# iclavera/learning_to_adapt

Hardware: AMD Instinct MI355X
Metric: controller-steps/sec (n_cand=2000, H=30, ens=5) (higher is better)
Workload: dtype f32

## Files before the change

include/l2a.h:

```cpp
#ifndef L2A_H_
#define L2A_H_

#ifdef __cplusplus
extern "C" {
#endif

typedef struct l2a_ctx l2a_ctx;
typedef struct l2a_model l2a_model;
typedef struct l2a_lstm l2a_lstm;
typedef struct l2a_reward_model l2a_reward_model;
typedef struct l2a_value_model l2a_value_model;
typedef struct l2a_policy_model l2a_policy_model;
typedef struct l2a_controller l2a_controller;

#define L2A_OK 0
#define L2A_EINVAL (-1)
#define L2A_EHIP (-2)
#define L2A_ENODEV (-3)
#define L2A_ESTATE (-4)
#define L2A_ESPLIT (-5)

#define L2A_ACT_IDENTITY 0
#define L2A_ACT_RELU 1
#define L2A_ACT_TANH 2
#define L2A_ACT_SIGMOID 3
#define L2A_ACT_SWISH 4

#define L2A_MODE_SINGLE 0
#define L2A_MODE_PER_BLOCK 1
#define L2A_MODE_MEAN 2

#define L2A_KERNEL_AUTO 0
#define L2A_KERNEL_MFMA 1
#define L2A_KERNEL_VALU 2

typedef struct l2a_reward {
    float w_vel;
    float inv_dt;
    float alive;
    float ctrl_coef;
    float dist_coef;
    int vel_index;
    int dist_index;
    int reserved;
} l2a_reward;

#define L2A_PROGRAM_MAX_TERMS 16
#define L2A_PROGRAM_MAX_CONSTS 64
#define L2A_SRC_OBS 0
#define L2A_SRC_ACT 1
#define L2A_SRC_NEXT 2
#define L2A_SRC_DELTA 3
#define L2A_TERM_LINEAR 0
#define L2A_TERM_SQSUM 1
#define L2A_TERM_NORM 2
#define L2A_TERM_INRANGE 3
typedef struct l2a_reward_term {
    int kind;
    int source;
    int index;
    int len;
    int target;
    float coef;
    float lo;
    float hi;
} l2a_reward_term;
typedef struct l2a_reward_program {
    int n_terms;
    int n_consts;
    float bias;
    int reserved;
    l2a_reward_term terms[L2A_PROGRAM_MAX_TERMS];
    float consts[L2A_PROGRAM_MAX_CONSTS];
} l2a_reward_program;

int l2a_init(int device, l2a_ctx** out);
void l2a_destroy(l2a_ctx* ctx);
const char* l2a_last_error(const l2a_ctx* ctx);
int l2a_device_info(const l2a_ctx* ctx, char* buf, int cap);
int l2a_set_kernel(l2a_ctx* ctx, int kind);
int l2a_set_split(l2a_ctx* ctx, int policy);
int l2a_set_batch(l2a_ctx* ctx, int sets);
int l2a_set_xcd_align(l2a_ctx* ctx, int on);
int l2a_set_fan(l2a_ctx* ctx, int on);
int l2a_set_double_rounds(l2a_ctx* ctx, int on);
int l2a_set_micro(l2a_ctx* ctx, int policy);
int l2a_launch_status(l2a_ctx* ctx, int* status_out);
int l2a_set_spin_limit(l2a_ctx* ctx, unsigned int polls);
int l2a_inject_status(l2a_ctx* ctx, int bits);
int l2a_set_debug_buffer(l2a_ctx* ctx, void* device_ptr);

int l2a_model_create(l2a_ctx* ctx, int obs_dim, int act_dim, int n_hidden, const int* hidden,
                     int hidden_act, int output_act, int n_sets, int mode, l2a_model** out);
void l2a_model_destroy(l2a_model* model);

int l2a_model_set_weights(l2a_model* model, int e, const void* const* device_ptrs,
                          void* stream);

int l2a_model_set_norm(l2a_model* model, int e, const double* mean_obs, const double* std_obs,
                       const double* mean_act, const double* std_act,
                       const double* mean_delta, const double* std_delta, void* stream);

int l2a_plan_rs(l2a_model* model, const float* obs0, const float* actions, int m, int n, int h,
                double discount, const l2a_reward* reward, int cand_offset, float* returns_out,
                unsigned long long* best_key, void* stream);

int l2a_plan_rs_sync(l2a_model* model, const float* obs_host, const float* actions, int m, int n, int h,
                     double discount, const l2a_reward* reward, int cand_offset, float* returns_out,
                     unsigned long long* keys_host_out, void* stream);

int l2a_plan_rs_chunk(l2a_model* model, const float* state, int state_per_row, const float* actions, int m, int n,
                      int h_chunk, int t0, double discount, const l2a_reward* reward, int cand_offset,
                      const float* returns_in, float* returns_out, float* state_out, unsigned long long* best_key,
                      void* stream);

int l2a_reward_program_check(const l2a_reward_program* program, int obs_dim, int act_dim);
int l2a_score_trajectory(l2a_ctx* ctx, const float* obs0, const float* traj, const float* actions, int m, int n, int h,
                         int obs_dim, int act_dim, double discount, const l2a_reward_program* program, int cand_offset,
                         float* returns_out, unsigned long long* best_key, void* stream);
int l2a_plan_rs_program(l2a_model* model, const float* obs0, const float* actions, int m, int n, int h, double discount,
                        const l2a_reward_program* program, int cand_offset, float* returns_out,
                        unsigned long long* best_key, float* traj_out, void* stream);

int l2a_reward_model_check(int obs_dim, int act_dim, int n_hidden, const int* hidden, int hidden_act);
int l2a_reward_model_geometry(int obs_dim, int act_dim, int n_hidden, const int* hidden, long long rows, int h, int num_cu,
                              int lds_per_block, int* out);
int l2a_reward_model_create(l2a_ctx* ctx, int obs_dim, int act_dim, int n_hidden, const int* hidden, int hidden_act,
                            l2a_reward_model** out);
void l2a_reward_model_destroy(l2a_reward_model* rm);
int l2a_reward_model_set_weights(l2a_reward_model* rm, const void* const* device_ptrs, void* stream);
int l2a_reward_model_set_norm(l2a_reward_model* rm, const double* mean_obs, const double* std_obs, const double* mean_act,
                              const double* std_act, const double* mean_delta, const double* std_delta, const double* mean_r,
                              const double* std_r, void* stream);
int l2a_reward_model_predict(l2a_reward_model* rm, const float* obs, const float* act, const float* next_obs, int rows,
                             float* rewards_out, void* stream);
int l2a_score_trajectory_model(l2a_reward_model* rm, const float* obs0, const float* traj, const float* actions, int m, int n,
                               int h, double discount, int cand_offset, float* returns_out, unsigned long long* best_key,
                               void* stream);
int l2a_plan_rs_reward_model(l2a_model* model, l2a_reward_model* rm, const float* obs0, const float* actions, int m, int n,
                             int h, double discount, int cand_offset, float* returns_out, unsigned long long* best_key,
                             float* traj_out, void* stream);

int l2a_value_model_check(int obs_dim, int n_hidden, const int* hidden, int hidden_act);
int l2a_value_model_geometry(int obs_dim, int n_hidden, const int* hidden, long long rows, int num_cu, int lds_per_block,
                             int* out);
int l2a_value_model_create(l2a_ctx* ctx, int obs_dim, int n_hidden, const int* hidden, int hidden_act, l2a_value_model** out);
void l2a_value_model_destroy(l2a_value_model* vm);
int l2a_value_model_set_weights(l2a_value_model* vm, const void* const* device_ptrs, void* stream);
int l2a_value_model_set_norm(l2a_value_model* vm, const double* mean_obs, const double* std_obs, const double* mean_v,
                             const double* std_v, void* stream);
int l2a_value_model_predict(l2a_value_model* vm, const float* states, int rows, float* values_out, void* stream);
int l2a_value_terminal(l2a_value_model* vm, const float* final_state, const float* returns_in, int m, int n, int h,
                       double discount, double value_coef, int cand_offset, float* returns_out, unsigned long long* best_key,
                       void* stream);
int l2a_plan_rs_value(l2a_model* model, l2a_value_model* vm, const float* obs0, const float* actions, int m, int n, int h,
                      double discount, const l2a_reward* reward, double value_coef, int cand_offset, float* returns_out,
                      unsigned long long* best_key, void* stream);
int l2a_plan_rs_program_value(l2a_model* model, l2a_value_model* vm, const float* obs0, const float* actions, int m, int n,
                              int h, double discount, const l2a_reward_program* program, double value_coef, int cand_offset,
                              float* returns_out, unsigned long long* best_key, float* traj_out, void* stream);
int l2a_plan_rs_reward_model_value(l2a_model* model, l2a_reward_model* rm, l2a_value_model* vm, const float* obs0,
                                   const float* actions, int m, int n, int h, double discount, double value_coef,
                                   int cand_offset, float* returns_out, unsigned long long* best_key, float* traj_out,
                                   void* stream);

int l2a_policy_model_check(int obs_dim, int act_dim, int n_hidden, const int* hidden, int hidden_act);
int l2a_policy_model_geometry(int obs_dim, int act_dim, int n_hidden, const int* hidden, long long rows, int num_cu,
                              int lds_per_block, int* out);
// ... 210 lines not shown
                                  const float* actions, int m, int n, int h, double discount, int cand_offset,
                                  float* returns_out, unsigned long long* best_key, float* traj_out, void* stream);
int l2a_lstm_traj_geometry(int obs_dim, int act_dim, int units, int m, int n, int h, int micro_policy, int num_cu, int* out);

#define L2A_STEP_MISS 1
#define L2A_STEP_UNSPLIT 2
#define L2A_STEP_DREW 3
int l2a_controller_create(l2a_model* model, int m, int n, int h, const double* low, const double* high, double discount,
                          const l2a_reward* reward, void* np_state_addr, int rng_threads, l2a_controller** out);
int l2a_lstm_controller_create(l2a_lstm* model, int m, int n, int h, const double* low, const double* high,
                               double discount, const l2a_reward* reward, void* np_state_addr, int rng_threads,
                               l2a_controller** out);
typedef int (*l2a_reduce_fn)(void* arg, unsigned long long* payload_dev, int words, void* stream);
int l2a_controller_create_sharded(l2a_model* model, int m, int n, int h, const double* low, const double* high,
                                  double discount, const l2a_reward* reward, void* np_state_addr, int rng_threads, int rank,
                                  int world, l2a_reduce_fn reduce, void* reduce_arg, l2a_controller** out);
int l2a_controller_create_sharded_device(l2a_model* model, int m, int n, int h, const double* low, const double* high,
                                         double discount, const l2a_reward* reward, unsigned long long seed, int rank, int world,
                                         l2a_reduce_fn reduce, void* reduce_arg, l2a_controller** out);
int l2a_lstm_controller_create_sharded(l2a_lstm* model, int m, int n, int h, const double* low, const double* high,
                                       double discount, const l2a_reward* reward, void* np_state_addr, int rng_threads, int rank,
                                       int world, l2a_reduce_fn reduce, void* reduce_arg, l2a_controller** out);
int l2a_lstm_controller_create_sharded_device(l2a_lstm* model, int m, int n, int h, const double* low, const double* high,
                                              double discount, const l2a_reward* reward, unsigned long long seed, int rank, int world,
                                              l2a_reduce_fn reduce, void* reduce_arg, l2a_controller** out);
int l2a_controller_create_device(l2a_model* model, int m, int n, int h, const double* low, const double* high, double discount,
                                 const l2a_reward* reward, unsigned long long seed, l2a_controller** out);
int l2a_lstm_controller_create_device(l2a_lstm* model, int m, int n, int h, const double* low, const double* high,
                                      double discount, const l2a_reward* reward, unsigned long long seed, l2a_controller** out);
int l2a_cem_controller_create_device(l2a_model* model, int m, int n, int h, const double* low, const double* high,
                                     double discount, const l2a_reward* reward, int iters, int num_elites, float alpha,
                                     int reference, unsigned long long seed, l2a_controller** out);
int l2a_cem_controller_create_sharded_device(l2a_model* model, int m, int n, int h, const double* low, const double* high,
                                             double discount, const l2a_reward* reward, int iters, int num_elites, float alpha,
                                             int reference, unsigned long long seed, int rank, int world, l2a_reduce_fn reduce,
                                             void* reduce_arg, l2a_controller** out);
int l2a_lstm_cem_controller_create_device(l2a_lstm* model, int m, int n, int h, const double* low, const double* high,
                                          double discount, const l2a_reward* reward, int iters, int num_elites, float alpha,
                                          int reference, unsigned long long seed, l2a_controller** out);
int l2a_lstm_cem_controller_create_sharded_device(l2a_lstm* model, int m, int n, int h, const double* low, const double* high,
                                                  double discount, const l2a_reward* reward, int iters, int num_elites, float alpha,
                                                  int reference, unsigned long long seed, int rank, int world, l2a_reduce_fn reduce,
                                                  void* reduce_arg, l2a_controller** out);
int l2a_cem_controller_result(l2a_controller* controller, float* mean_out, float* std_out, float* returns_out);
int l2a_mppi_controller_create_device(l2a_model* model, int m, int n, int h, const double* low, const double* high,
                                      double discount, const l2a_reward* reward, int iters, float kappa, float beta,
                                      const double* sigma, unsigned long long seed, l2a_controller** out);
int l2a_mppi_controller_create_sharded_device(l2a_model* model, int m, int n, int h, const double* low, const double* high,
                                              double discount, const l2a_reward* reward, int iters, float kappa, float beta,
                                              const double* sigma, unsigned long long seed, int rank, int world,
                                              l2a_reduce_fn reduce, void* reduce_arg, l2a_controller** out);
int l2a_mppi_controller_reset(l2a_controller* controller, const unsigned char* dones);
int l2a_mppi_controller_reseed(l2a_controller* controller, unsigned long long seed);
int l2a_mppi_controller_result(l2a_controller* controller, float* mean_out, float* ess_out, int* valid_out, float* returns_out);
int l2a_icem_controller_create_device(l2a_model* model, int m, int n, int h, const double* low, const double* high,
                                      double discount, const l2a_reward* reward, int iters, const int* pops, int K, int Kk,
                                      float alpha, float rho, const double* sigma0, int add_mean, unsigned long long seed,
                                      l2a_controller** out);
int l2a_icem_controller_create_sharded_device(l2a_model* model, int m, int n, int h, const double* low, const double* high,
                                              double discount, const l2a_reward* reward, int iters, const int* pops, int K, int Kk,
                                              float alpha, float rho, const double* sigma0, int add_mean, unsigned long long seed,
                                              int rank, int world, l2a_reduce_fn reduce, void* reduce_arg, l2a_controller** out);
int l2a_icem_controller_reset(l2a_controller* controller, const unsigned char* dones);
int l2a_icem_controller_reseed(l2a_controller* controller, unsigned long long seed);
int l2a_icem_controller_result(l2a_controller* controller, float* mean_out, float* std_out, float* kept_out, int* kc_out,
                               float* heads_out, float* returns_out);
int l2a_icem_controller_set_noise(l2a_controller* controller, const float* M_host);
void l2a_controller_destroy(l2a_controller* controller);
int l2a_controller_step(l2a_controller* controller, const double* obs, double* action_out, long long* index_out,
                        float* return_out, void* stream);
int l2a_lstm_controller_step(l2a_controller* controller, const double* obs, const float* c0, const float* h0,
                             float* c_next, float* h_next, double* action_out, long long* index_out, float* return_out,
                             void* stream);
int l2a_controller_begin(l2a_controller* controller, const double* obs, void* stream);
int l2a_lstm_controller_begin(l2a_controller* controller, const double* obs, const float* c0, const float* h0,
                              float* c_next, float* h_next, void* stream);
int l2a_controller_finish(l2a_controller* controller, double* action_out, long long* index_out, float* return_out);
int l2a_controller_rearm(l2a_controller* controller);
const float* l2a_controller_actions(const l2a_controller* controller);
int l2a_controller_stats(l2a_controller* controller, double* out, int cap);

int l2a_plan_geometry(int obs_dim, int act_dim, int n_hidden, const int* hidden, int n_sets, int mode, int m, int n, int h,
                      const int* policy, int* out);
int l2a_lstm_plan_geometry(int obs_dim, int act_dim, int n_layers, const int* units, int cell_type, int m, int n, int h, int request,
                           const int* policy, int* out);
int l2a_mfma_eligible(int obs_dim, int act_dim, int n_hidden, const int* hidden);
long long l2a_packed_layer_floats(int k_in, int n_out);
int l2a_pack_layer_host(const float* w, int k_in, int n_out, float* out);
long long l2a_micro_layout_floats(int obs_dim, int act_dim, int n_hidden, int hidden);
int l2a_micro_pack_layer_host(const float* w, int obs_dim, int act_dim, int n_hidden, int hidden, int layer, float* out);

#ifdef __cplusplus
}
#endif
#endif
```

learning_to_adapt_amd/_lib.py:

```python

import ctypes
import json
import os

from .envs.reward_spec import RewardProgram, RewardSpec
from .envs.termination import TerminationProgram

_HERE = os.path.dirname(os.path.abspath(__file__))
LIB_PATH = os.environ.get("L2A_LIB_PATH") or os.path.join(_HERE, "libl2a_hip.so")

L2A_OK = 0
L2A_EINVAL = -1
L2A_ESTATE = -4
L2A_ESPLIT = -5
L2A_STEP_MISS = 1
L2A_STEP_UNSPLIT = 2
L2A_STEP_DREW = 3
ACT_CODES = {None: 0, "identity": 0, "relu": 1, "tanh": 2, "sigmoid": 3, "swish": 4}
MODE_CODES = {"single": 0, "per_block": 1, "mean": 2}
KERNEL_CODES = {"auto": 0, "mfma": 1, "valu": 2}
CELL_CODES = {"lstm": 0, "gru": 1, "rnn": 2}

EXPORTED_SYMBOLS = (
    "l2a_init", "l2a_destroy", "l2a_last_error", "l2a_device_info", "l2a_set_kernel", "l2a_set_split", "l2a_set_batch", "l2a_set_xcd_align", "l2a_set_fan", "l2a_set_double_rounds", "l2a_set_micro",
    "l2a_launch_status", "l2a_set_debug_buffer", "l2a_set_spin_limit", "l2a_inject_status",
    "l2a_model_create", "l2a_model_destroy", "l2a_model_set_weights", "l2a_model_set_weights_strided",
    "l2a_model_set_norm", "l2a_model_adapt_sgd", "l2a_model_adapt_sgd_host", "l2a_model_adapt_sgd_raw", "l2a_model_get_weights",
    "l2a_plan_rs", "l2a_plan_rs_sync", "l2a_plan_rs_chunk", "l2a_reward_program_check", "l2a_score_trajectory", "l2a_plan_rs_program",
    "l2a_reward_model_check", "l2a_reward_model_geometry", "l2a_reward_model_create", "l2a_reward_model_destroy", "l2a_reward_model_set_weights", "l2a_reward_model_set_norm",
    "l2a_reward_model_predict", "l2a_score_trajectory_model", "l2a_plan_rs_reward_model", "l2a_predict", "l2a_key_encode", "l2a_key_decode", "l2a_mfma_eligible", "l2a_plan_geometry",
    "l2a_packed_layer_floats", "l2a_pack_layer_host", "l2a_micro_layout_floats", "l2a_micro_pack_layer_host",
    "l2a_comm_unique_id", "l2a_comm_init", "l2a_comm_destroy", "l2a_allreduce_best", "l2a_plan_payload",
    "l2a_cem_sample", "l2a_cem_refit", "l2a_cem_pick", "l2a_cem_refit_sample", "l2a_cem_refit_sample_fused",
    "l2a_mppi_sample", "l2a_mppi_update", "l2a_mppi_sample_shard",
    "l2a_icem_sample", "l2a_icem_refit",
    "l2a_mppi_controller_create_device", "l2a_mppi_controller_create_sharded_device", "l2a_mppi_controller_reset",
    "l2a_mppi_controller_reseed", "l2a_mppi_controller_result",
    "l2a_icem_sample_shard", "l2a_icem_controller_create_device", "l2a_icem_controller_create_sharded_device", "l2a_icem_controller_reset",
    "l2a_icem_controller_reseed", "l2a_icem_controller_result",
    "l2a_icem_noise_matrix", "l2a_icem_sample_noise", "l2a_icem_sample_noise_shard", "l2a_icem_controller_set_noise",
    "l2a_lstm_create", "l2a_rnn_create", "l2a_lstm_destroy", "l2a_lstm_set_weights", "l2a_lstm_set_norm", "l2a_lstm_plan_rs", "l2a_lstm_plan_rs_sync", "l2a_lstm_plan_rs_chunk",
    "l2a_lstm_predict", "l2a_lstm_advance", "l2a_lstm_mfma_eligible",
    "l2a_lstm_rollout_traj", "l2a_lstm_plan_rs_program", "l2a_lstm_plan_rs_reward_model", "l2a_lstm_traj_geometry", "l2a_lstm_plan_geometry",
    "l2a_rollout_traj", "l2a_mlp_traj_geometry",
    "l2a_value_model_check", "l2a_value_model_geometry", "l2a_value_model_create", "l2a_value_model_destroy", "l2a_value_model_set_weights",
    "l2a_value_model_set_norm", "l2a_value_model_predict", "l2a_value_terminal", "l2a_plan_rs_value", "l2a_plan_rs_program_value",
    "l2a_plan_rs_reward_model_value",
    "l2a_policy_model_check", "l2a_policy_model_geometry", "l2a_policy_model_create", "l2a_policy_model_destroy",
    "l2a_policy_model_set_weights", "l2a_policy_model_set_norm", "l2a_policy_act", "l2a_policy_propose",
    "l2a_termination_check", "l2a_score_trajectory_term", "l2a_plan_rs_term",
    "l2a_particle_score", "l2a_plan_rs_particles", "l2a_plan_rs_particles_program", "l2a_plan_rs_particles_reward_model",
    "l2a_particle_perm", "l2a_particle_shuffle", "l2a_plan_rs_particles_ts1",
    "l2a_particle_step", "l2a_plan_rs_particles_ts1_program", "l2a_plan_rs_particles_ts1_reward_model",
    "l2a_controller_create", "l2a_controller_create_sharded", "l2a_controller_create_sharded_device", "l2a_lstm_controller_create", "l2a_controller_create_device", "l2a_lstm_controller_create_device",
    "l2a_lstm_controller_create_sharded", "l2a_lstm_controller_create_sharded_device",
    "l2a_controller_destroy", "l2a_controller_step", "l2a_controller_begin", "l2a_lstm_controller_begin", "l2a_controller_finish",
    "l2a_lstm_controller_step", "l2a_controller_rearm", "l2a_controller_actions", "l2a_controller_stats",
    "l2a_cem_controller_create_device", "l2a_cem_controller_result",
    "l2a_cem_shard_pack", "l2a_cem_shard_unpack", "l2a_cem_word_encode", "l2a_cem_word_decode", "l2a_cem_controller_create_sharded_device",
    "l2a_cem_pick_act", "l2a_lstm_cem_controller_create_device", "l2a_lstm_cem_controller_create_sharded_device",
)


class L2AError(RuntimeError):
    pass


def lstm_traj_geometry(obs_dim, act_dim, units, m, n, h, micro=1, cus=0):
    lib = load()
    out = (ctypes.c_int * 8)()
    rc = lib.l2a_lstm_traj_geometry(int(obs_dim), int(act_dim), int(units), int(m), int(n), int(h), int(micro), int(cus), out)
    if rc != L2A_OK:
        raise L2AError("l2a_lstm_traj_geometry failed (%d)" % rc)
    v = list(out)
    return dict(single=bool(v[0]), launches=v[1], workgroups=v[2], workgroups_per_env=v[3], micro_tiles=v[4], full_workgroups=v[5])


def mlp_traj_geometry(obs_dim, act_dim, n_hidden, hidden, mode, n_sets, m, n, h, micro=1, cus=0):
    lib = load()
    out = (ctypes.c_int * 8)()
    rc = lib.l2a_mlp_traj_geometry(int(obs_dim), int(act_dim), int(n_hidden), int(hidden), MODE_CODES[mode], int(n_sets), int(m), int(n),
                                   int(h), int(micro), int(cus), out)
    if rc != L2A_OK:
        raise L2AError("l2a_mlp_traj_geometry failed (%d)" % rc)
    v = list(out)
    return dict(single=bool(v[0]), launches=v[1], workgroups=v[2], workgroups_per_env=v[3], micro_tiles=v[4], full_workgroups=v[5])


def plan_geometry(obs_dim, act_dim, hidden, n_sets, mode, m, n, h, split=-1, fan=-1, micro=-1, cus=0, double=-1):
    lib = load()
    hid = (ctypes.c_int * len(hidden))(*[int(x) for x in hidden])
    pol = (ctypes.c_int * 5)(int(split), int(fan), int(micro), int(cus), int(double))
    out = (ctypes.c_int * 12)()
    rc = lib.l2a_plan_geometry(int(obs_dim), int(act_dim), len(hidden), hid, int(n_sets), MODE_CODES[mode], int(m), int(n), int(h), pol, out)
    if rc != L2A_OK:
        raise L2AError("l2a_plan_geometry failed (%d)" % rc)
    v = list(out)
    return dict(kernel=("valu", "mfma16", "micro")[v[0]], nt=v[1], split=v[2], split_from=v[3], fan=bool(v[4]), workgroups=v[5],
                lds_bytes=v[6], sets_per_batch=v[7], micro_tiles=v[8], placement_units=v[9], front_workgroups=v[10],
                whole_instance=bool(v[11]))


LSTM_FAMILIES = ("lstm_valu", "lstm_mfma16", "lstm_micro", "lstm_micro_traj", "generic_valu", "generic_mfma16", "generic_micro")
LSTM_REQUEST_BITS = {"per_row": 1, "state_out": 2, "no_results": 4, "no_split": 8, "traj": 16}


def lstm_plan_geometry(obs_dim, act_dim, units, cell, m, n, h, request=(), kernel="auto", split=-1, micro=-1, cus=0, lds=0):
    lib = load()
    layers = [int(units)] if isinstance(units, int) else [int(x) for x in units]
    arr = (ctypes.c_int * len(layers))(*layers)
    pol = (ctypes.c_int * 5)(KERNEL_CODES[kernel], int(split), int(micro), int(cus), int(lds))
    out = (ctypes.c_int * 12)()
    rc = lib.l2a_lstm_plan_geometry(int(obs_dim), int(act_dim), 0 if isinstance(units, int) else len(layers), arr, CELL_CODES[cell],
                                    int(m), int(n), int(h), sum(LSTM_REQUEST_BITS[r] for r in request), pol, out)
    if rc != L2A_OK:
        raise L2AError("l2a_lstm_plan_geometry failed (%d)" % rc)
    v = list(out)
    return dict(family=LSTM_FAMILIES[v[0]], mtm=v[1], split=v[2], workgroups=v[3], lds_bytes=v[4], tiles_per_env=v[5], mc_w=v[6],
                mc_hi=v[7], mc_r=v[8], exchange_bytes=v[9], publish=bool(v[10]))


def reward_model_check(obs_dim, act_dim, hidden, hidden_act):
    lib = load()
    hid = (ctypes.c_int * max(len(hidden), 1))(*[int(x) for x in hidden])
    code = hidden_act if isinstance(hidden_act, int) else ACT_CODES.get(hidden_act, -1)
    rc = lib.l2a_reward_model_check(int(obs_dim), int(act_dim), len(hidden), hid, int(code))
    return None if rc == L2A_OK else lib.l2a_last_error(None).decode()


def reward_model_geometry(obs_dim, act_dim, hidden, rows, h, cus=0, lds_per_block=160 * 1024):
    lib = load()
    hid = (ctypes.c_int * max(len(hidden), 1))(*[int(x) for x in hidden])
    out = (ctypes.c_int * 8)()
    rc = lib.l2a_reward_model_geometry(int(obs_dim), int(act_dim), len(hidden), hid, int(rows), int(h), int(cus), int(lds_per_block), out)
    if rc != L2A_OK:
        raise L2AError("l2a_reward_model_geometry failed (%d): %s" % (rc, lib.l2a_last_error(None).decode()))
    v = list(out)
    return dict(RT=v[0], CT=v[1], S=v[2], workgroups=v[3], passes=v[4], lds_bytes=v[5])


def value_model_check(obs_dim, hidden, hidden_act):
    lib = load()
    hid = (ctypes.c_int * max(len(hidden), 1))(*[int(x) for x in hidden])
    code = hidden_act if isinstance(hidden_act, int) else ACT_CODES.get(hidden_act, -1)
    rc = lib.l2a_value_model_check(int(obs_dim), len(hidden), hid, int(code))
    return None if rc == L2A_OK else lib.l2a_last_error(None).decode()


def value_model_geometry(obs_dim, hidden, rows, cus=0, lds_per_block=160 * 1024):
    lib = load()
    hid = (ctypes.c_int * max(len(hidden), 1))(*[int(x) for x in hidden])
    out = (ctypes.c_int * 8)()
    rc = lib.l2a_value_model_geometry(int(obs_dim), len(hidden), hid, int(rows), int(cus), int(lds_per_block), out)
    if rc != L2A_OK:
        raise L2AError("l2a_value_model_geometry failed (%d): %s" % (rc, lib.l2a_last_error(None).decode()))
    v = list(out)
    return dict(RT=v[0], workgroups=v[1], lds_bytes=v[2])


def _policy_symbols(lib):
    if not hasattr(lib, "l2a_policy_model_create"):
        raise L2AError("the loaded library (%s) has no l2a_policy_model_* entries: it predates policy priors - rebuild it" % LIB_PATH)


def policy_model_check(obs_dim, act_dim, hidden, hidden_act):
    lib = load()
    _policy_symbols(lib)
    hid = (ctypes.c_int * max(len(hidden), 1))(*[int(x) for x in hidden])
    code = hidden_act if isinstance(hidden_act, int) else ACT_CODES.get(hidden_act, -1)
    rc = lib.l2a_policy_model_check(int(obs_dim), int(act_dim), len(hidden), hid, int(code))
    return None if rc == L2A_OK else lib.l2a_last_error(None).decode()


def policy_model_geometry(obs_dim, act_dim, hidden, rows, cus=0, lds_per_block=160 * 1024):
    lib = load()
    _policy_symbols(lib)
    hid = (ctypes.c_int * max(len(hidden), 1))(*[int(x) for x in hidden])
    out = (ctypes.c_int * 8)()
    rc = lib.l2a_policy_model_geometry(int(obs_dim), int(act_dim), len(hidden), hid, int(rows), int(cus), int(lds_per_block), out)
    if rc != L2A_OK:
        raise L2AError("l2a_policy_model_geometry failed (%d): %s" % (rc, lib.l2a_last_error(None).decode()))
    v = list(out)
    return dict(RT=v[0], workgroups=v[1], lds_bytes=v[2])


_lib = None


def load():
    global _lib
    if _lib is not None:
        return _lib
    if not os.path.exists(LIB_PATH):
        raise L2AError(
            "%s not found - build it with `python -c 'import __graft_entry__ as g; g.build()'` "
            "(hipcc --offload-arch=gfx950); there is no CPU fallback" % LIB_PATH)
    try:
        import torch
    except ImportError:
        pass
    lib = ctypes.CDLL(LIB_PATH)
    c = ctypes
    vp, i32, f32 = c.c_void_p, c.c_int, c.c_float
    lib.l2a_init.argtypes = [i32, c.POINTER(vp)]
    lib.l2a_init.restype = i32
    lib.l2a_destroy.argtypes = [vp]
    lib.l2a_destroy.restype = None
    lib.l2a_last_error.argtypes = [vp]
    lib.l2a_last_error.restype = c.c_char_p
    lib.l2a_device_info.argtypes = [vp, c.c_char_p, i32]
    lib.l2a_device_info.restype = i32
    lib.l2a_set_kernel.argtypes = [vp, i32]
    lib.l2a_set_kernel.restype = i32
    lib.l2a_set_split.argtypes = [vp, i32]
    lib.l2a_set_split.restype = i32
    if os.environ.get("L2A_LIB_PATH") and not hasattr(lib, "l2a_set_batch"):
        lib.l2a_set_batch = lambda handle, sets: 0
    else:
        lib.l2a_set_batch.argtypes = [vp, i32]
        lib.l2a_set_batch.restype = i32
    if os.environ.get("L2A_LIB_PATH") and not hasattr(lib, "l2a_set_micro"):
        lib.l2a_set_micro = lambda handle, policy: 0
    else:
        lib.l2a_set_micro.argtypes = [vp, i32]
        lib.l2a_set_micro.restype = i32
    if os.environ.get("L2A_LIB_PATH") and not hasattr(lib, "l2a_set_fan"):
        lib.l2a_set_fan = lambda handle, on: 0
    else:
        lib.l2a_set_fan.argtypes = [vp, i32]
        lib.l2a_set_fan.restype = i32
    if os.environ.get("L2A_LIB_PATH") and not hasattr(lib, "l2a_set_double_rounds"):
        lib.l2a_set_double_rounds = lambda handle, on: 0
    else:
        lib.l2a_set_double_rounds.argtypes = [vp, i32]
        lib.l2a_set_double_rounds.restype = i32
    if os.environ.get("L2A_LIB_PATH") and not hasattr(lib, "l2a_set_xcd_align"):
        lib.l2a_set_xcd_align = lambda handle, on: 0
    else:
        lib.l2a_set_xcd_align.argtypes = [vp, i32]
        lib.l2a_set_xcd_align.restype = i32
    lib.l2a_launch_status.argtypes = [vp, c.POINTER(i32)]
    lib.l2a_launch_status.restype = i32
    lib.l2a_set_debug_buffer.argtypes = [vp, vp]
    lib.l2a_set_debug_buffer.restype = i32
    lib.l2a_set_spin_limit.argtypes = [vp, c.c_uint]
    lib.l2a_set_spin_limit.restype = i32
    lib.l2a_inject_status.argtypes = [vp, i32]
    lib.l2a_inject_status.restype = i32
    lib.l2a_model_create.argtypes = [vp, i32, i32, i32, c.POINTER(i32), i32, i32, i32, i32, c.POINTER(vp)]
    lib.l2a_model_create.restype = i32
    lib.l2a_model_destroy.argtypes = [vp]
    lib.l2a_model_destroy.restype = None
    lib.l2a_model_set_weights.argtypes = [vp, i32, c.POINTER(vp), vp]
    lib.l2a_model_set_weights.restype = i32
    lib.l2a_model_set_weights_strided.argtypes = [vp, i32, i32, c.POINTER(vp), c.POINTER(c.c_longlong), vp]
    lib.l2a_model_set_weights_strided.restype = i32
    lib.l2a_model_adapt_sgd.argtypes = [vp, c.POINTER(vp), vp, vp, i32, i32, f32, vp]
    lib.l2a_model_adapt_sgd.restype = i32
    lib.l2a_model_adapt_sgd_host.argtypes = [vp, c.POINTER(vp), vp, vp, i32, i32, f32, vp]
    lib.l2a_model_adapt_sgd_host.restype = i32
    lib.l2a_model_adapt_sgd_raw.argtypes = [vp, c.POINTER(vp), vp, vp, vp, vp, vp, vp, vp, vp, vp, i32, i32, f32, vp]
    lib.l2a_model_adapt_sgd_raw.restype = i32
    lib.l2a_model_get_weights.argtypes = [vp, i32, c.POINTER(vp), vp]
    lib.l2a_model_get_weights.restype = i32
    dp = c.POINTER(c.c_double)
    lib.l2a_model_set_norm.argtypes = [vp, i32, dp, dp, dp, dp, dp, dp, vp]
    lib.l2a_model_set_norm.restype = i32
    lib.l2a_plan_rs.argtypes = [vp, vp, vp, i32, i32, i32, c.c_double, c.POINTER(RewardSpec), i32, vp, vp, vp]
    lib.l2a_plan_rs.restype = i32
    lib.l2a_plan_rs_sync.argtypes = [vp, vp, vp, i32, i32, i32, c.c_double, c.POINTER(RewardSpec), i32, vp, vp, vp]
    lib.l2a_plan_rs_sync.restype = i32
    lib.l2a_plan_rs_chunk.argtypes = [vp, vp, i32, vp, i32, i32, i32, i32, c.c_double, c.POINTER(RewardSpec), i32, vp, vp, vp, vp, vp]
    lib.l2a_plan_rs_chunk.restype = i32
    lib.l2a_reward_program_check.argtypes = [c.POINTER(RewardProgram), i32, i32]
    lib.l2a_reward_program_check.restype = i32
    lib.l2a_score_trajectory.argtypes = [vp, vp, vp, vp, i32, i32, i32, i32, i32, c.c_double, c.POINTER(RewardProgram), i32, vp, vp, vp]
    lib.l2a_score_trajectory.restype = i32
    lib.l2a_plan_rs_program.argtypes = [vp, vp, vp, i32, i32, i32, c.c_double, c.POINTER(RewardProgram), i32, vp, vp, vp, vp]
    lib.l2a_plan_rs_program.restype = i32
    if hasattr(lib, "l2a_termination_check"):
        tp = c.POINTER(TerminationProgram)
        lib.l2a_termination_check.argtypes = [tp, i32]
        lib.l2a_termination_check.restype = i32
        lib.l2a_score_trajectory_term.argtypes = [vp, vp, vp, vp, vp, i32, i32, i32, i32, i32, c.c_double, c.POINTER(RewardProgram), tp,
                                                  vp, c.c_double, i32, vp, vp, vp, vp]
        lib.l2a_score_trajectory_term.restype = i32
        lib.l2a_plan_rs_term.argtypes = [vp, vp, vp, vp, vp, i32, i32, i32, c.c_double, c.POINTER(RewardProgram), tp, c.c_double, i32,
                                         vp, vp, vp, vp, vp]
        lib.l2a_plan_rs_term.restype = i32
    if hasattr(lib, "l2a_value_model_create"):
        dbl = c.c_double
        lib.l2a_value_model_check.argtypes = [i32, i32, c.POINTER(i32), i32]
        lib.l2a_value_model_check.restype = i32
        lib.l2a_value_model_geometry.argtypes = [i32, i32, c.POINTER(i32), c.c_longlong, i32, i32, c.POINTER(i32)]
        lib.l2a_value_model_geometry.restype = i32
        lib.l2a_value_model_create.argtypes = [vp, i32, i32, c.POINTER(i32), i32, c.POINTER(vp)]
        lib.l2a_value_model_create.restype = i32
        lib.l2a_value_model_destroy.argtypes = [vp]
        lib.l2a_value_model_destroy.restype = None
        lib.l2a_value_model_set_weights.argtypes = [vp, c.POINTER(vp), vp]
        lib.l2a_value_model_set_weights.restype = i32
        lib.l2a_value_model_set_norm.argtypes = [vp, dp, dp, dp, dp, vp]
        lib.l2a_value_model_set_norm.restype = i32
        lib.l2a_value_model_predict.argtypes = [vp, vp, i32, vp, vp]
        lib.l2a_value_model_predict.restype = i32
        lib.l2a_value_terminal.argtypes = [vp, vp, vp, i32, i32, i32, dbl, dbl, i32, vp, vp, vp]
        lib.l2a_value_terminal.restype = i32
        lib.l2a_plan_rs_value.argtypes = [vp, vp, vp, vp, i32, i32, i32, dbl, c.POINTER(RewardSpec), dbl, i32, vp, vp, vp]
        lib.l2a_plan_rs_value.restype = i32
        lib.l2a_plan_rs_program_value.argtypes = [vp, vp, vp, vp, i32, i32, i32, dbl, c.POINTER(RewardProgram), dbl, i32, vp, vp, vp, vp]
        lib.l2a_plan_rs_program_value.restype = i32
        lib.l2a_plan_rs_reward_model_value.argtypes = [vp, vp, vp, vp, vp, i32, i32, i32, dbl, dbl, i32, vp, vp, vp, vp]
        lib.l2a_plan_rs_reward_model_value.restype = i32
    if hasattr(lib, "l2a_policy_model_create"):
        u64 = c.c_ulonglong
        lib.l2a_policy_model_check.argtypes = [i32, i32, i32, c.POINTER(i32), i32]
        lib.l2a_policy_model_check.restype = i32
        lib.l2a_policy_model_geometry.argtypes = [i32, i32, i32, c.POINTER(i32), c.c_longlong, i32, i32, c.POINTER(i32)]
        lib.l2a_policy_model_geometry.restype = i32
        lib.l2a_policy_model_create.argtypes = [vp, i32, i32, i32, c.POINTER(i32), i32, c.POINTER(vp)]
        lib.l2a_policy_model_create.restype = i32
        lib.l2a_policy_model_destroy.argtypes = [vp]
        lib.l2a_policy_model_destroy.restype = None
        lib.l2a_policy_model_set_weights.argtypes = [vp, c.POINTER(vp), vp]
        lib.l2a_policy_model_set_weights.restype = i32
        lib.l2a_policy_model_set_norm.argtypes = [vp, dp, dp, dp, dp, vp]
        lib.l2a_policy_model_set_norm.restype = i32
        lib.l2a_policy_act.argtypes = [vp, vp, i32, vp, u64, u64, vp, vp, vp, vp, vp]
        lib.l2a_policy_act.restype = i32
        lib.l2a_policy_propose.argtypes = [vp, vp, vp, i32, i32, i32, i32, i32, vp, u64, u64, vp, vp, vp, vp, vp, i32, vp]
        lib.l2a_policy_propose.restype = i32
    if hasattr(lib, "l2a_reward_model_create"):
        lib.l2a_reward_model_check.argtypes = [i32, i32, i32, c.POINTER(i32), i32]
        lib.l2a_reward_model_check.restype = i32
        if hasattr(lib, "l2a_reward_model_geometry"):
            lib.l2a_reward_model_geometry.argtypes = [i32, i32, i32, c.POINTER(i32), c.c_longlong, i32, i32, i32, c.POINTER(i32)]
            lib.l2a_reward_model_geometry.restype = i32
        lib.l2a_reward_model_create.argtypes = [vp, i32, i32, i32, c.POINTER(i32), i32, c.POINTER(vp)]
        lib.l2a_reward_model_create.restype = i32
        lib.l2a_reward_model_destroy.argtypes = [vp]
        lib.l2a_reward_model_destroy.restype = None
        lib.l2a_reward_model_set_weights.argtypes = [vp, c.POINTER(vp), vp]
        lib.l2a_reward_model_set_weights.restype = i32
        lib.l2a_reward_model_set_norm.argtypes = [vp, dp, dp, dp, dp, dp, dp, dp, dp, vp]
        lib.l2a_reward_model_set_norm.restype = i32
        lib.l2a_reward_model_predict.argtypes = [vp, vp, vp, vp, i32, vp, vp]
        lib.l2a_reward_model_predict.restype = i32
        lib.l2a_score_trajectory_model.argtypes = [vp, vp, vp, vp, i32, i32, i32, c.c_double, i32, vp, vp, vp]
        lib.l2a_score_trajectory_model.restype = i32
        lib.l2a_plan_rs_reward_model.argtypes = [vp, vp, vp, vp, i32, i32, i32, c.c_double, i32, vp, vp, vp, vp]
        lib.l2a_plan_rs_reward_model.restype = i32
    lib.l2a_predict.argtypes = [vp, vp, vp, i32, i32, vp, vp]
    lib.l2a_predict.restype = i32
    lib.l2a_key_encode.argtypes = [f32, i32]
    lib.l2a_key_encode.restype = c.c_ulonglong
    lib.l2a_key_decode.argtypes = [c.c_ulonglong, c.POINTER(f32), c.POINTER(i32)]
    lib.l2a_key_decode.restype = None
    lib.l2a_mfma_eligible.argtypes = [i32, i32, i32, c.POINTER(i32)]
    lib.l2a_mfma_eligible.restype = i32
    lib.l2a_plan_geometry.argtypes = [i32, i32, i32, c.POINTER(i32), i32, i32, i32, i32, i32, c.POINTER(i32), c.POINTER(i32)]
    lib.l2a_plan_geometry.restype = i32
    lib.l2a_packed_layer_floats.argtypes = [i32, i32]
    lib.l2a_packed_layer_floats.restype = c.c_longlong
    lib.l2a_pack_layer_host.argtypes = [c.POINTER(f32), i32, i32, c.POINTER(f32)]
    lib.l2a_pack_layer_host.restype = i32
    if hasattr(lib, "l2a_micro_layout_floats"):
        lib.l2a_micro_layout_floats.argtypes = [i32, i32, i32, i32]
        lib.l2a_micro_layout_floats.restype = c.c_longlong
        lib.l2a_micro_pack_layer_host.argtypes = [c.POINTER(f32), i32, i32, i32, i32, i32, c.POINTER(f32)]
        lib.l2a_micro_pack_layer_host.restype = i32
    lib.l2a_comm_unique_id.argtypes = [c.c_char_p]
    lib.l2a_comm_unique_id.restype = i32
    lib.l2a_comm_init.argtypes = [vp, i32, i32, c.c_char_p]
    lib.l2a_comm_init.restype = i32
    lib.l2a_comm_destroy.argtypes = [vp]
    lib.l2a_comm_destroy.restype = i32
    lib.l2a_allreduce_best.argtypes = [vp, vp, i32, vp]
    lib.l2a_allreduce_best.restype = i32
    lib.l2a_lstm_create.argtypes = [vp, i32, i32, i32, i32, i32, c.POINTER(vp)]
    lib.l2a_lstm_create.restype = i32
    lib.l2a_rnn_create.argtypes = [vp, i32, i32, i32, c.POINTER(i32), i32, i32, i32, c.POINTER(vp)]
    lib.l2a_rnn_create.restype = i32
    lib.l2a_lstm_destroy.argtypes = [vp]
    lib.l2a_lstm_destroy.restype = None
    lib.l2a_lstm_set_weights.argtypes = [vp, c.POINTER(vp), vp]
    lib.l2a_lstm_set_weights.restype = i32
    lib.l2a_lstm_set_norm.argtypes = [vp, dp, dp, dp, dp, dp, dp, vp]
    lib.l2a_lstm_set_norm.restype = i32
    lib.l2a_lstm_plan_rs.argtypes = [vp, vp, vp, vp, vp, i32, i32, i32, c.c_double, c.POINTER(RewardSpec), i32, vp, vp, vp]
    lib.l2a_lstm_plan_rs.restype = i32
    lib.l2a_cem_sample.argtypes = [vp, vp, c.c_ulonglong, c.c_ulonglong, vp, vp, vp, vp, i32, i32, i32, i32, i32, i32, i32,
                                   vp, vp, vp, vp]
    lib.l2a_cem_sample.restype = i32
    lib.l2a_cem_refit.argtypes = [vp, vp, vp, i32, i32, i32, i32, i32, f32, vp, vp, vp, vp]
    lib.l2a_cem_refit.restype = i32
    lib.l2a_cem_pick.argtypes = [vp, vp, vp, vp, vp, i32, i32, i32, i32, i32, vp, vp]
    lib.l2a_cem_pick.restype = i32
    if hasattr(lib, "l2a_cem_refit_sample"):
        lib.l2a_cem_refit_sample.argtypes = [vp, vp, vp, i32, i32, i32, i32, i32, i32, f32, vp, c.c_ulonglong, c.c_ulonglong, vp, vp,
                                             i32, i32, vp, vp, vp, vp, vp, vp, vp, vp]
        lib.l2a_cem_refit_sample.restype = i32
        lib.l2a_cem_refit_sample_fused.argtypes = [vp, i32, i32, i32, i32, i32, i32]
        lib.l2a_cem_refit_sample_fused.restype = i32
    if hasattr(lib, "l2a_mppi_sample"):
        lib.l2a_mppi_sample.argtypes = [vp, vp, c.c_ulonglong, c.c_ulonglong, vp, vp, vp, f32, vp, vp, i32, i32, i32, i32, vp, vp, vp, vp]
        lib.l2a_mppi_sample.restype = i32
        lib.l2a_mppi_update.argtypes = [vp, vp, vp, i32, i32, i32, i32, f32, vp, vp, vp]
        lib.l2a_mppi_update.restype = i32
    if hasattr(lib, "l2a_icem_sample"):
        lib.l2a_icem_sample.argtypes = [vp, vp, c.c_ulonglong, c.c_ulonglong, vp, vp, vp, vp, vp, vp, f32, vp, vp, i32, i32, i32, i32, i32,
                                        i32, vp, vp, vp, vp, vp]
        lib.l2a_icem_sample.restype = i32
        lib.l2a_icem_refit.argtypes = [vp, vp, vp, vp, vp, i32, i32, i32, i32, i32, i32, f32, vp, vp, vp, vp, vp, vp, vp]
        lib.l2a_icem_refit.restype = i32
    lib.l2a_lstm_plan_rs_sync.argtypes = [vp, vp, vp, vp, vp, i32, i32, i32, c.c_double, c.POINTER(RewardSpec), i32, vp, vp, vp, vp]
    lib.l2a_lstm_plan_rs_sync.restype = i32
    lib.l2a_lstm_plan_rs_chunk.argtypes = [vp, vp, vp, vp, i32, vp, i32, i32, i32, i32, c.c_double, c.POINTER(RewardSpec), i32,
                                           vp, vp, vp, vp, vp, vp, vp]
    lib.l2a_lstm_plan_rs_chunk.restype = i32
    lib.l2a_lstm_predict.argtypes = [vp, vp, vp, vp, vp, i32, vp, vp, vp, vp]
    lib.l2a_lstm_predict.restype = i32
    if hasattr(lib, "l2a_lstm_advance"):
        lib.l2a_lstm_advance.argtypes = [vp, vp, vp, vp, vp, i32, vp, vp, vp]
        lib.l2a_lstm_advance.restype = i32
    if os.environ.get("L2A_LIB_PATH") and not hasattr(lib, "l2a_plan_payload"):
        pass
    else:
        lib.l2a_plan_payload.argtypes = [vp, vp, i32, c.c_ulonglong, vp, vp]
        lib.l2a_plan_payload.restype = i32
    lib.l2a_lstm_mfma_eligible.argtypes = [i32, i32, i32]
    lib.l2a_lstm_mfma_eligible.restype = i32
    if hasattr(lib, "l2a_lstm_rollout_traj"):
        lib.l2a_lstm_rollout_traj.argtypes = [vp, vp, vp, vp, vp, i32, i32, i32, i32, vp, vp]
        lib.l2a_lstm_rollout_traj.restype = i32
        lib.l2a_lstm_plan_rs_program.argtypes = [vp, vp, vp, vp, vp, i32, i32, i32, c.c_double, c.POINTER(RewardProgram), i32, vp, vp, vp, vp]
        lib.l2a_lstm_plan_rs_program.restype = i32
        lib.l2a_lstm_plan_rs_reward_model.argtypes = [vp, vp, vp, vp, vp, vp, i32, i32, i32, c.c_double, i32, vp, vp, vp, vp]
        lib.l2a_lstm_plan_rs_reward_model.restype = i32
        lib.l2a_lstm_traj_geometry.argtypes = [i32, i32, i32, i32, i32, i32, i32, i32, c.POINTER(i32)]
        lib.l2a_lstm_traj_geometry.restype = i32
    if hasattr(lib, "l2a_lstm_plan_geometry"):
        lib.l2a_lstm_plan_geometry.argtypes = [i32, i32, i32, c.POINTER(i32), i32, i32, i32, i32, i32, c.POINTER(i32), c.POINTER(i32)]
        lib.l2a_lstm_plan_geometry.restype = i32
    if hasattr(lib, "l2a_rollout_traj"):
# ... 123 lines not shown
                                                                  i32, f32, f32, vp, i32, c.c_ulonglong, i32, i32, vp, vp, c.POINTER(vp)]
        lib.l2a_icem_controller_create_sharded_device.restype = i32
        lib.l2a_icem_controller_reset.argtypes = [vp, vp]
        lib.l2a_icem_controller_reset.restype = i32
        lib.l2a_icem_controller_reseed.argtypes = [vp, c.c_ulonglong]
        lib.l2a_icem_controller_reseed.restype = i32
        lib.l2a_icem_controller_result.argtypes = [vp, vp, vp, vp, vp, vp, vp]
        lib.l2a_icem_controller_result.restype = i32
    if hasattr(lib, "l2a_icem_sample_noise"):
        lib.l2a_icem_noise_matrix.argtypes = [i32, c.c_double, vp]
        lib.l2a_icem_noise_matrix.restype = i32
        lib.l2a_icem_sample_noise.argtypes = [vp, vp, c.c_ulonglong, c.c_ulonglong, vp, vp, vp, vp, vp, vp, vp, vp, vp, i32, i32, i32, i32,
                                              i32, i32, vp, vp, vp, vp, vp]
        lib.l2a_icem_sample_noise.restype = i32
        lib.l2a_icem_sample_noise_shard.argtypes = [vp, vp, c.c_ulonglong, c.c_ulonglong, vp, vp, vp, vp, vp, vp, vp, vp, vp, i32, i32, i32,
                                                    i32, i32, i32, i32, i32, vp, vp, vp, vp, vp]
        lib.l2a_icem_sample_noise_shard.restype = i32
        lib.l2a_icem_controller_set_noise.argtypes = [vp, vp]
        lib.l2a_icem_controller_set_noise.restype = i32
    _lib = lib
    return lib


def key_decode(key):
    lib = load()
    ret, idx = ctypes.c_float(), ctypes.c_int()
    lib.l2a_key_decode(ctypes.c_ulonglong(int(key) & 0xFFFFFFFFFFFFFFFF), ctypes.byref(ret), ctypes.byref(idx))
    return ret.value, idx.value


class Context(object):

    _by_device = {}

    def __init__(self, device=0):
        self.lib = load()
        handle = ctypes.c_void_p()
        rc = self.lib.l2a_init(int(device), ctypes.byref(handle))
        if rc != L2A_OK:
            raise L2AError("l2a_init(device=%d) failed (%d): %s" % (
                device, rc, self.lib.l2a_last_error(None).decode()))
        self.handle = handle
        self.device = int(device)
        self.pid = os.getpid()

    @classmethod
    def get(cls, device=0):
        ctx = cls._by_device.get(device)
        if ctx is None or ctx.pid != os.getpid():
            ctx = cls(device)
            cls._by_device[device] = ctx
            kind = os.environ.get("L2A_KERNEL")
            if kind:
                ctx.set_kernel(kind)
        return ctx

    def check(self, rc, what):
        if rc != L2A_OK:
            raise L2AError("%s failed (%d): %s" % (what, rc, self.lib.l2a_last_error(self.handle).decode()))

    def info(self):
        buf = ctypes.create_string_buffer(512)
        self.check(self.lib.l2a_device_info(self.handle, buf, 512), "l2a_device_info")
        return json.loads(buf.value.decode())

    def set_kernel(self, kind):
        self.check(self.lib.l2a_set_kernel(self.handle, KERNEL_CODES[kind]), "l2a_set_kernel")

    def set_split(self, policy):
        self.check(self.lib.l2a_set_split(self.handle, int(policy)), "l2a_set_split")

    def set_batch(self, sets):
        self.check(self.lib.l2a_set_batch(self.handle, int(sets)), "l2a_set_batch")

    def set_micro(self, policy):
        self.check(self.lib.l2a_set_micro(self.handle, int(policy)), "l2a_set_micro")

    def set_xcd_align(self, on):
        self.check(self.lib.l2a_set_xcd_align(self.handle, int(bool(on))), "l2a_set_xcd_align")

    def set_fan(self, on):
        self.check(self.lib.l2a_set_fan(self.handle, int(bool(on))), "l2a_set_fan")

    def set_double_rounds(self, on):
        self.check(self.lib.l2a_set_double_rounds(self.handle, int(bool(on))), "l2a_set_double_rounds")

    def launch_status_value(self):
        st = ctypes.c_int()
        self.check(self.lib.l2a_launch_status(self.handle, ctypes.byref(st)), "l2a_launch_status")
        return st.value

    def launch_status(self):
        st = self.launch_status_value()
        if st != 0:
            raise L2AError("rollout launch reported status 0x%x (member-split exchange timed out; "
                           "set L2A_SPLIT=0 to disable the split)" % st)
        return st

    def check_or_degrade(self):
        st = self.launch_status_value()
        if st == 0:
            return True
        if getattr(self, "split_degraded", False):
            raise L2AError("rollout launch reported status 0x%x with the tile split disabled" % st)
        self.set_split(0)
        self.split_degraded = True
        return False

    def force_unsplit(self):
        self.launch_status_value()
        if not getattr(self, "split_degraded", False):
            self.set_split(0)
            self.split_degraded = True

    def plan_payload(self, best_key, m, digest, payload, stream_ptr):
        assert best_key.is_cuda and payload.is_cuda and str(best_key.dtype) == "torch.int64" and str(payload.dtype) == "torch.int64"
        assert best_key.numel() == m and payload.numel() == m + 3
        rc = self.lib.l2a_plan_payload(self.handle, ctypes.c_void_p(best_key.data_ptr()), int(m), ctypes.c_ulonglong(int(digest)),
                                       ctypes.c_void_p(payload.data_ptr()), stream_ptr)
        self.check(rc, "l2a_plan_payload")

    def score_trajectory(self, obs0, traj, actions, m, n, h, discount, program, cand_offset=0, returns_out=None,
                         best_key=None, stream_ptr=None):
        import torch
        assert isinstance(program, RewardProgram)
        for t in (obs0, traj, actions):
            assert t.is_cuda and t.dtype == torch.float32 and t.is_contiguous()
        obs_dim, act_dim = int(obs0.shape[-1]), int(actions.shape[-1])
        assert obs0.numel() == m * obs_dim and traj.numel() == h * m * n * obs_dim and actions.numel() == h * m * n * act_dim
        if returns_out is not None:
            assert returns_out.is_cuda and returns_out.dtype == torch.float32 and returns_out.numel() == m * n
        if best_key is not None:
            assert best_key.is_cuda and best_key.dtype == torch.int64 and best_key.numel() == m
        if stream_ptr is None:
            stream_ptr = ctypes.c_void_p(torch.cuda.current_stream(obs0.device).cuda_stream)
        ptr = lambda t: ctypes.c_void_p(t.data_ptr()) if t is not None else ctypes.c_void_p(0)
        rc = self.lib.l2a_score_trajectory(self.handle, ptr(obs0), ptr(traj), ptr(actions), int(m), int(n), int(h), obs_dim,
                                           act_dim, float(discount), ctypes.byref(program), int(cand_offset), ptr(returns_out),
                                           ptr(best_key), stream_ptr)
        self.check(rc, "l2a_score_trajectory")

    def score_trajectory_term(self, obs0, traj, actions, m, n, h, discount, termination, program=None, step_rewards=None,
                              terminal_values=None, value_coef=1.0, cand_offset=0, returns_out=None, steps_alive_out=None,
                              best_key=None, stream_ptr=None):
        import torch
        assert isinstance(termination, TerminationProgram)
        assert program is None or isinstance(program, RewardProgram)
        assert traj.is_cuda and traj.dtype == torch.float32 and traj.is_contiguous()
        obs_dim = int(traj.shape[-1])
        assert traj.numel() == h * m * n * obs_dim
        act_dim = int(actions.shape[-1]) if actions is not None else 1
        if program is not None:
            for t in (obs0, actions):
                assert t.is_cuda and t.dtype == torch.float32 and t.is_contiguous()
            assert obs0.numel() == m * obs_dim and actions.numel() == h * m * n * act_dim
        if step_rewards is not None:
            assert step_rewards.is_cuda and step_rewards.dtype == torch.float32 and step_rewards.is_contiguous()
            assert step_rewards.numel() == h * m * n
        if terminal_values is not None:
            assert terminal_values.is_cuda and terminal_values.dtype == torch.float32 and terminal_values.is_contiguous()
            assert terminal_values.numel() == m * n
        if returns_out is not None:
            assert returns_out.is_cuda and returns_out.dtype == torch.float32 and returns_out.numel() == m * n
        if steps_alive_out is not None:
            assert steps_alive_out.is_cuda and steps_alive_out.dtype == torch.int32 and steps_alive_out.numel() == m * n
        if best_key is not None:
# ... 14 lines not shown
```

learning_to_adapt_amd/csrc/build.py:

```python

import os
import shutil
import subprocess
import sys
from concurrent.futures import ThreadPoolExecutor

HERE = os.path.dirname(os.path.abspath(__file__))
PKG = os.path.dirname(HERE)
OUT = os.path.join(PKG, "libl2a_hip.so")
RNG_OUT = os.path.join(PKG, "libl2a_rng.so")
OBJ_DIR = os.path.join(HERE, "_obj")
HEADERS = ["l2a_host.h", "l2a_kernels.h", "l2a_valu.h", "l2a_adapt.h", "l2a_mfma.h", "l2a_mfma_launch.h", "l2a_lstm.h",
           "l2a_lstm_valu.h", "l2a_rnn_valu.h", "l2a_rnn_mfma.h", "l2a_lstm_launch.h", "l2a_micro.h", "l2a_rnn_micro.h", "l2a_micro_pack.h", "l2a_rm_layer.h", "l2a_micro_launch.h", "l2a_rng.h", os.path.join("..", "..", "include", "l2a.h")]
SOURCES = ["l2a_api.hip", "l2a_mfma_inst.hip", "l2a_lstm_api.hip", "l2a_lstm_inst.hip", "l2a_micro_inst.hip", "l2a_micro_traj_inst.hip", "l2a_mlp_micro_traj_inst.hip", "l2a_rnn_micro_inst.hip", "l2a_comm.hip", "l2a_cem.hip", "l2a_mppi.hip", "l2a_icem.hip", "l2a_step.hip", "l2a_score.hip", "l2a_score_mlp.hip", "l2a_value.hip", "l2a_policy.hip", "l2a_particles.hip", "l2a_particle_step.hip", "l2a_rng.c"]
INSTANCES = [(1, 2), (1, 4), (1, 8), (2, 2), (2, 4)]
FAN_INSTANCES = [(1, 2), (1, 4), (1, 8), (2, 8)]
WHOLE_INSTANCES = [(2, 8), (1, 8)]
LSTM_INSTANCES = [2, 4, 8]
FLAGS = ["--offload-arch=gfx950", "-O3", "-std=c++17", "-fPIC"]
KERNEL_FLAGS = ["-mllvm", "--amdgpu-mfma-vgpr-form"]
LSTM_FLAGS = []
MICRO_FLAGS = []
SCORE_FLAGS = ["-ffp-contract=off"]


def _hipcc():
    exe = shutil.which("hipcc") or "/opt/rocm/bin/hipcc"
    if not os.path.exists(exe):
        raise RuntimeError("hipcc not found (looked on PATH and in /opt/rocm/bin)")
    return exe


def build_rng(verbose=True):
    gcc = shutil.which("gcc") or shutil.which("clang") or ("/opt/rocm/lib/llvm/bin/clang" if os.path.exists("/opt/rocm/lib/llvm/bin/clang") else None)
    if gcc is None:
        if verbose:
            print("[l2a] no C compiler found: libl2a_rng.so cannot be built")
        return None
    subprocess.check_call([gcc, "-O3", "-fPIC", "-shared", "-ffp-contract=off", "-pthread",
                           os.path.join(HERE, "l2a_rng.c"), "-o", RNG_OUT, "-lm"])
    return RNG_OUT


def _obj_fresh(obj):
    dep = obj[:-2] + ".d"
    if not os.path.exists(obj) or not os.path.exists(dep):
        return False
    t = os.path.getmtime(obj)
    with open(dep) as f:
        words = f.read().replace("\\\n", " ").split()
    files = [w for w in words[1:] if not w.endswith(":")]
    own = [w for w in files if not w.startswith("/opt/") and not w.startswith("/usr/")]
    return all(os.path.exists(w) and os.path.getmtime(w) <= t for w in own + [os.path.abspath(__file__)])


def up_to_date():
    if not os.path.exists(OUT) or (shutil.which("gcc") and not os.path.exists(RNG_OUT)):
        return False
    t = os.path.getmtime(OUT)
    if os.path.isdir(OBJ_DIR) and os.listdir(OBJ_DIR):
        if not all(_obj_fresh(os.path.join(OBJ_DIR, o)) and os.path.getmtime(os.path.join(OBJ_DIR, o)) <= t for o in unit_table()):
            return False
        return os.path.getmtime(os.path.join(HERE, "l2a_rng.c")) <= os.path.getmtime(RNG_OUT) if os.path.exists(RNG_OUT) else True
    deps = [os.path.join(HERE, f) for f in SOURCES + HEADERS] + [os.path.abspath(__file__)]
    return all(os.path.getmtime(d) <= t for d in deps)


def _compile(job):
    src, obj, defs = job
    cmd = [_hipcc()] + FLAGS + defs + ["-MD", "-MF", obj[:-2] + ".d", "-c", os.path.join(HERE, src), "-o", obj]
    subprocess.check_call(cmd, cwd=HERE)
    return obj


def unit_table():
    t = {"l2a_api.o": ("l2a_api.hip", []),
         "l2a_lstm_api.o": ("l2a_lstm_api.hip", KERNEL_FLAGS),
         "l2a_comm.o": ("l2a_comm.hip", []),
         "l2a_cem.o": ("l2a_cem.hip", []),
         "l2a_mppi.o": ("l2a_mppi.hip", SCORE_FLAGS),
         "l2a_icem.o": ("l2a_icem.hip", []),
         "l2a_step.o": ("l2a_step.hip", []),
         "l2a_score.o": ("l2a_score.hip", SCORE_FLAGS),
         "l2a_score_mlp.o": ("l2a_score_mlp.hip", SCORE_FLAGS),
         "l2a_value.o": ("l2a_value.hip", SCORE_FLAGS),
         "l2a_policy.o": ("l2a_policy.hip", SCORE_FLAGS),
         "l2a_particles.o": ("l2a_particles.hip", SCORE_FLAGS),
         "l2a_particle_step.o": ("l2a_particle_step.hip", SCORE_FLAGS),
         "l2a_micro.o": ("l2a_micro_inst.hip", MICRO_FLAGS),
         "l2a_micro_traj.o": ("l2a_micro_traj_inst.hip", MICRO_FLAGS),
         "l2a_mlp_micro_traj.o": ("l2a_mlp_micro_traj_inst.hip", MICRO_FLAGS),
         "l2a_rnn_micro.o": ("l2a_rnn_micro_inst.hip", MICRO_FLAGS)}
    for utw in LSTM_INSTANCES:
        t["l2a_lstm_%d.o" % utw] = ("l2a_lstm_inst.hip", ["-DL2A_INST_UTW=%d" % utw] + LSTM_FLAGS)
    for nt, tpw in INSTANCES:
        t["l2a_mfma_%d_%d.o" % (nt, tpw)] = ("l2a_mfma_inst.hip", ["-DL2A_INST_NT=%d" % nt, "-DL2A_INST_TPW=%d" % tpw] +
                                               (KERNEL_FLAGS if nt == 1 else []))
    for nt, tpw in FAN_INSTANCES:
        t["l2a_mfma_fan_%d_%d.o" % (nt, tpw)] = ("l2a_mfma_inst.hip", ["-DL2A_INST_NT=%d" % nt, "-DL2A_INST_TPW=%d" % tpw,
                                                                        "-DL2A_INST_FAN=1"] + KERNEL_FLAGS)
    for nt, tpw in WHOLE_INSTANCES:
        t["l2a_mfma_whole_%d_%d.o" % (nt, tpw)] = ("l2a_mfma_inst.hip", ["-DL2A_INST_NT=%d" % nt, "-DL2A_INST_TPW=%d" % tpw,
                                                                          "-DL2A_INST_FAN=2"] + KERNEL_FLAGS)
    return t


def link(objs, out):
    if not os.path.exists(RNG_OUT) or os.path.getmtime(RNG_OUT) < os.path.getmtime(os.path.join(HERE, "l2a_rng.c")):
        build_rng(verbose=False)
    if not os.path.exists(RNG_OUT):
        raise RuntimeError("libl2a_rng.so could not be built (no gcc / clang): libl2a_hip.so links against it")
    subprocess.check_call([_hipcc(), "--offload-arch=gfx950", "-shared", "-fPIC", "-o", out] + objs +
                          ["-L" + PKG, "-ll2a_rng", "-Wl,-rpath,$ORIGIN", "-ldl"], cwd=HERE)
    return out


def relink(units, verbose=True):
    table = unit_table()
    jobs = [(table[u][0], os.path.join(OBJ_DIR, u), table[u][1]) for u in units]
    with ThreadPoolExecutor(max_workers=max(1, len(jobs))) as pool:
        list(pool.map(_compile, jobs))
    return link([os.path.join(OBJ_DIR, o) for o in table], OUT)


def variant(name, units, defs):
    table = unit_table()
    jobs, objs = [], []
    for o, (src, flags) in table.items():
        if o in units:
            vo = os.path.join(OBJ_DIR, o[:-2] + "_" + name + ".o")
            jobs.append((src, vo, flags + list(defs)))
            objs.append(vo)
        else:
            objs.append(os.path.join(OBJ_DIR, o))
    with ThreadPoolExecutor(max_workers=max(1, len(jobs))) as pool:
        list(pool.map(_compile, jobs))
    return link(objs, os.path.join(PKG, "libl2a_hip_%s.so" % name))


def build(force=False, verbose=True, only=None):
    if not force and only is None and up_to_date():
        if verbose:
            print("[l2a] %s is up to date" % OUT)
        return OUT
    os.makedirs(OBJ_DIR, exist_ok=True)
    table = unit_table()
    jobs = []
    for o, (src, flags) in table.items():
        obj = os.path.join(OBJ_DIR, o)
        if only is not None and o.startswith("l2a_mfma_") and os.path.exists(obj) and \
                tuple(int(x) for x in o[len("l2a_mfma_"):-2].replace("fan_", "").replace("whole_", "").split("_")) not in only:
            continue
        if not force and only is None and _obj_fresh(obj):
            continue
        jobs.append((src, obj, flags))
    if verbose:
        print("[l2a] hipcc %s : %d of %d translation units, %d parallel jobs"
              % (" ".join(FLAGS), len(jobs), len(table), min(max(len(jobs), 1), os.cpu_count() or 1)))
    if jobs:
        with ThreadPoolExecutor(max_workers=min(len(jobs), os.cpu_count() or 1)) as pool:
            list(pool.map(_compile, jobs))
    build_rng(verbose)
    link([os.path.join(OBJ_DIR, o) for o in table], OUT)
    return OUT


if __name__ == "__main__":
    only = None
    for a in sys.argv[1:]:
        if a.startswith("--units="):
            relink([u if u.endswith(".o") else u + ".o" for u in a[len("--units="):].split(",")])
            sys.exit(0)
        if a.startswith("--only="):
            only = [tuple(int(x) for x in part.split("x")) for part in a[len("--only="):].split(",")]
    build(force="--force" in sys.argv, only=only)
```

learning_to_adapt_amd/csrc/l2a_api.hip:

```cpp

#define L2A_PACK_KERNELS 1
#include "l2a_host.h"
#include "l2a_kernels.h"
#include "l2a_valu.h"
#include "l2a_adapt.h"
#include "l2a_mfma_launch.h"
#include "l2a_micro_pack.h"
#include "l2a_micro_launch.h"

#include <chrono>
#include <cmath>
#include <cstdio>
#include <cstdlib>
#include <cstring>
#include <string>
#include <vector>

#include <immintrin.h>
#include <unistd.h>

namespace {

std::string g_init_error;

// ... 2 lines not shown
int l2a_fail(const l2a_ctx* ctx, int code, const std::string& msg) {
    if (ctx) ctx->err = msg; else g_init_error = msg;
    return code;
}

struct l2a_mlp_shape {
    int obs_dim = 0, act_dim = 0, in_dim = 0;
    int n_hidden = 0;
    int hidden[L2A_MAX_LAYERS] = {0};
    int hidden_act = L2A_ACT_RELU, output_act = L2A_ACT_IDENTITY;
    int n_sets = 1, mode = L2A_MODE_SINGLE;
    bool mfma_ok = false;
    int H = 0, TPW = 0, KG0 = 0, OT = 0, hmax = 0;
    long long set_stride = 0;
    bool micro_ok = false;
    int m_o4 = 0;
};

struct l2a_model : l2a_mlp_shape {
    l2a_ctx* ctx = nullptr;
    float* wblk = nullptr;
    long long raw_w[L2A_MAX_LAYERS] = {0};
    long long raw_b[L2A_MAX_LAYERS] = {0};
    long long pk_w0 = 0, pk_wmid = 0, pk_wmid_stride = 0, pk_wout = 0, pk_bout = 0, nm_off = 0;
    long long pk_m = 0;
    std::vector<char> weights_set, norm_set;
    std::vector<std::vector<float>> norm_stage;
    l2a_xbuf xb;
    float* adapt_scratch = nullptr;
    long long adapt_scratch_floats = 0;
    float* prog_buf = nullptr;
    long long prog_buf_floats = 0;
    float* value_buf = nullptr;
    long long value_buf_floats = 0;
    float* pol_buf = nullptr;
    long long pol_buf_floats = 0;
    float* term_buf = nullptr;
    long long term_buf_floats = 0;
    float* part_buf = nullptr;
    long long part_buf_floats = 0;
    struct adapt_slot {
        float* stage_host = nullptr;
        float* stage_dev = nullptr;
        long long stage_floats = 0;
        hipEvent_t done = nullptr;
        bool pending = false;
    } aslot[2];
    int aslot_next = 0;
};

namespace {

inline bool fast_act(int a) { return a == L2A_ACT_RELU || a == L2A_ACT_IDENTITY; }

inline int fail(const l2a_ctx* ctx, int code, const std::string& msg) { return l2a_fail(ctx, code, msg); }

inline int ceil_div(int a, int b) { return (a + b - 1) / b; }

bool mfma_eligible(int obs_dim, int act_dim, int n_hidden, const int* hidden) {
    if (n_hidden < 1 || n_hidden > L2A_MAX_LAYERS - 1) return false;
    const int H = hidden[0];
    if (H != 128 && H != 256 && H != 512) return false;
    for (int i = 1; i < n_hidden; ++i)
        if (hidden[i] != H) return false;
    if (obs_dim < 1 || obs_dim > 16 * L2A_OTMAX) return false;
    if (act_dim < 1 || act_dim > 16) return false;
    if (obs_dim + act_dim > 16 * L2A_KG0MAX) return false;
    return true;
}

long long packed_floats(int k_in, int n_out) {
    return (long long)ceil_div(n_out, 16) * ceil_div(k_in, 16) * 256;
}

template <typename K>
int allow_big_lds(const l2a_ctx* ctx, K kernel, int bytes) {
    L2A_HIP(ctx, hipFuncSetAttribute(reinterpret_cast<const void*>(kernel),
                                     hipFuncAttributeMaxDynamicSharedMemorySize, bytes));
    return L2A_OK;
}


struct l2a_rollout_policy {
    int kernel_kind, split_policy, fan_policy, double_policy, micro_policy, batch_sets, xcd_align;
    int num_cu, lds_per_block;
    int force_nt;
    bool dbg_front;
};

l2a_rollout_policy rollout_policy(const l2a_ctx* ctx) {
    static const int force_nt = [] { const char* e = std::getenv("L2A_FORCE_NT"); return (e && (e[0] == '1' || e[0] == '2')) ? e[0] - '0' : 0; }();
    static const bool dbg_front = [] { const char* e = std::getenv("L2A_DBG_FRONT"); return e && e[0] == '1'; }();
    return {ctx->kernel_kind, ctx->split_policy, ctx->fan_policy, ctx->double_policy, ctx->micro_policy, ctx->batch_sets,
            ctx->xcd_align, ctx->num_cu > 0 ? ctx->num_cu : 256, ctx->lds_per_block, force_nt, dbg_front};
}

struct l2a_rollout_request {
    int mode, m, n, h;
    bool obs_per_row, state_out, results;
};

enum { L2A_FAMILY_VALU = 0, L2A_FAMILY_MFMA16 = 1, L2A_FAMILY_MICRO = 2 };

struct l2a_rollout_launch {
    int family;
    int nt, geo, gact;
    unsigned grid;
    int smem;
    int c_lo, c_hi, sa_elems, tiles_per_env, cst_set, n_cst, lb, cst_off;
    int split, split_from;
    int pl_units, pl_f, pl_r, pl_w;
    int mc_w, mc_hi, mc_r;
    long long m_bytes;
};

struct l2a_rollout_plan {
    int n_launch;
    l2a_rollout_launch launch[2];
    int done_total;
    long long xbuf_bytes;
};

int split_mode_for(const l2a_mlp_shape& md, int policy, int e_loop) {
    if (policy == 0) return 0;
    if ((e_loop & 1) && md.n_hidden >= 2 && policy == 1) return 2;
    return (e_loop >= 2) ? 1 : 0;
}

int choose_nt(const l2a_mlp_shape& md, const l2a_rollout_policy& pol, int m, int n, int e_loop, int sa_bytes_nt2, int other_bytes_nt2) {
    const int cus = pol.num_cu;
    if (2 * sa_bytes_nt2 + other_bytes_nt2 > pol.lds_per_block) return 1;
    if (md.TPW >= 8 || md.OT >= 4) return 1;
    if (pol.force_nt) return pol.force_nt;
    const long long wg1 = (long long)m * ceil_div(n, 16);
    const long long wg2 = (long long)m * ceil_div(n, 32);
    const long long t = wg1 % cus;
    double cost1 = (double)((wg1 + cus - 1) / cus);
    if (wg1 > cus && t != 0 && 2 * t <= cus && split_mode_for(md, pol.split_policy, e_loop) != 0) cost1 = (double)(wg1 / cus) + 0.8;
    const double cost2 = (double)((wg2 + cus - 1) / cus) * 1.9;
    return (cost2 < cost1) ? 2 : 1;
}

int sa_elems_for(const l2a_mlp_shape& md, int nt) {
    const int ht = md.H / 16;
    const int a = nt * ht;
    const int b = L2A_NW * nt * md.OT;
    return (a > b ? a : b) * 64;
}

int plan_rollout(const l2a_mlp_shape& md, const l2a_rollout_policy& pol, const l2a_rollout_request& rq, l2a_rollout_plan* plan,
                 std::string* err) {
    auto bad = [err](int code, const std::string& msg) { *err = msg; return code; };
    *plan = l2a_rollout_plan();
    plan->n_launch = 1;
    if (rq.mode == L2A_MODE_PER_BLOCK && rq.m > md.n_sets)
        return bad(L2A_EINVAL, "per-block mode needs one weight set per env/block");
    int kind = pol.kernel_kind;
    if (kind == L2A_KERNEL_AUTO) kind = md.mfma_ok ? L2A_KERNEL_MFMA : L2A_KERNEL_VALU;
    if (kind == L2A_KERNEL_MFMA && !md.mfma_ok)
        return bad(L2A_EINVAL, "model shape is not eligible for the MFMA kernel "
                               "(needs equal hidden widths of 128/256/512, obs_dim<=64, act_dim<=16)");
    if (kind != L2A_KERNEL_MFMA) {
        l2a_rollout_launch& d = plan->launch[0];
        d.family = L2A_FAMILY_VALU;
        d.c_hi = rq.n;
        d.tiles_per_env = ceil_div(rq.n, L2A_VT);
        d.smem = (md.in_dim + 2 * md.hmax + 3 * md.obs_dim + md.act_dim + 1) * L2A_VT * 4;
        if (d.smem > pol.lds_per_block)
            return bad(L2A_EINVAL, "LDS budget exceeded by the VALU kernel (" + std::to_string(d.smem) + " B)");
        d.grid = (unsigned)(rq.m * d.tiles_per_env);
        return L2A_OK;
    }

    const int e_loop = (rq.mode == L2A_MODE_MEAN) ? md.n_sets : 1;
    const int cus = pol.num_cu;
    const int cst_set = 32 * md.KG0 + 48 * md.OT + md.n_hidden * md.H;
    const bool gact = !(fast_act(md.hidden_act) && fast_act(md.output_act));
// ... 55 lines not shown
    if (md.micro_ok && pol.micro_policy != 0) {
        const long long tiles16 = (long long)rq.m * ceil_div(n_rest, 16);
        const l2a_micro_deal deal = l2a_deal_micro(cus, rq.m, n_rest, 3);
        const int smem_need = l2a_mlp_micro_smem(md.H, md.KG0, md.n_hidden, e_loop);
        const long long span = (long long)((rq.mode == L2A_MODE_PER_BLOCK ? rq.m : e_loop) - 1) * md.set_stride * 4 +
                               l2a_mlp_micro_floats(md.H, md.KG0, md.n_hidden) * 4;
        const bool eligible = !rq.obs_per_row && !rq.state_out && deal.hi <= 3 && rq.results &&
                              smem_need <= pol.lds_per_block && span < (1LL << 31);
        const bool unfilled = 2 * tiles16 > cus && tiles16 < cus;
        const bool small_one_set = e_loop == 1 && 2 * tiles16 <= cus;
        const bool wanted = pol.micro_policy == 2 || (pol.micro_policy == 1 && md.H == 512 && (unfilled || small_one_set));
        if (eligible && wanted) {
            d.family = L2A_FAMILY_MICRO;
            d.gact = (gact || md.n_hidden == 1) ? 1 : 0;
            d.grid = (unsigned)(rq.m * deal.W);
            d.smem = smem_need < 84 * 1024 ? 84 * 1024 : smem_need;
            d.mc_w = deal.W; d.mc_hi = deal.hi; d.mc_r = deal.mc_r;
            d.m_bytes = span;
            if (front_k) plan->done_total = (int)(front.grid + d.grid);
            return L2A_OK;
        }
    }

    d.family = L2A_FAMILY_MFMA16;
    d.gact = gact ? 1 : 0;
    int nt = choose_nt(md, pol, rq.m, n_rest, e_loop, sa_elems_for(md, 2) * 16, e_loop * cst_set * 4 + 4 * md.OT * 64 * 16);
    int fan_nt = 0;
    if (!front_k && pol.split_policy != 0 && pol.fan_policy != 0 && rq.h < 4096 && rq.mode == L2A_MODE_MEAN && e_loop >= 3 && e_loop <= 8) {
        if ((long long)rq.m * ceil_div(rq.n, 16) * e_loop <= cus) fan_nt = 1;
        else if (md.TPW == 8 && md.OT <= 3 && (long long)rq.m * ceil_div(rq.n, 32) * e_loop <= cus &&
                 2 * sa_elems_for(md, 2) * 16 + cst_set * 4 + e_loop * 2 * md.OT * 64 * 16 <= pol.lds_per_block)
            fan_nt = 2;
    }
    const bool fan = fan_nt != 0;
    if (fan) nt = fan_nt;
    d.nt = nt;
    d.sa_elems = sa_elems_for(md, nt);
    d.tiles_per_env = ceil_div(n_rest, 16 * nt);
    d.cst_set = cst_set;
    const long long pairs = (long long)rq.m * d.tiles_per_env;
    d.split_from = -1;
    long long split_pairs = 0;
    const int split_mode = split_mode_for(md, pol.split_policy, e_loop);
    if (fan) {
        d.split = 3;
        split_pairs = pairs;
    } else if (pol.split_policy != 0 && nt == 1 && rq.h < 4096) {
        if (2 * pairs <= cus) {
            d.split = split_mode;
            split_pairs = d.split ? pairs : 0;
        } else if (pairs > cus && pairs % cus != 0 && 2 * (pairs % cus) <= cus && split_mode != 0) {
            d.split = split_mode;
            split_pairs = pairs % cus;
            d.split_from = (int)(pairs - split_pairs);
        }
    }
    if (d.split) plan->xbuf_bytes = split_pairs * (fan ? e_loop : 4) * 2 * (long long)(nt * md.OT * 2 * 64 * 16);
    const bool uniform_split = d.split && d.split_from < 0;
    const int nseq = fan ? 1 : uniform_split ? (e_loop + 1) / 2 : e_loop;
    const int x_bytes = (fan ? e_loop : 2) * nt * md.OT * 64 * 16;
    d.n_cst = nseq;
    d.smem = lds_plan(nt, nseq, x_bytes, &d.lb, &d.cst_off);
    if (d.smem > pol.lds_per_block)
        return bad(L2A_EINVAL, "LDS budget exceeded (" + std::to_string(d.smem) + " B)");
    long long n_wg = fan ? pairs * e_loop : pairs + (d.split ? split_pairs : 0);
    if (pol.xcd_align && d.split_from < 0 && n_wg <= cus) {
        int units = 0;
        long long w = 0;
        if (rq.mode == L2A_MODE_PER_BLOCK) { units = rq.m; w = (long long)d.tiles_per_env * (d.split ? 2 : 1); }
        else if (fan) { units = e_loop; w = pairs; }
        else if (d.split && e_loop > 1) { units = 2; w = pairs; }
        if (units >= 2 && units <= 8) {
            const int f = 8 / units;
            const long long slots = (w + f - 1) / f;
            if (8 * slots <= cus) {
                d.pl_units = units; d.pl_f = f; d.pl_r = 8 - units * f; d.pl_w = (int)w;
                n_wg = 8 * slots;
            }
        }
    }
    d.grid = (unsigned)n_wg;
    const bool whole1 = !fan && pol.double_policy != 0 && e_loop == 1 && nt == 1 && md.TPW == 8 && md.OT <= 3 &&
                        d.split == 0 && d.split_from < 0;
    d.geo = fan ? 1 : whole1 ? 2 : 0;
    if (front_k) plan->done_total = (int)(front.grid + pairs);
    return L2A_OK;
}

struct l2a_traj_plan {
    bool single;
    l2a_micro_deal deal;
    int gact, smem;
    long long m_bytes;
};

l2a_traj_plan plan_traj_rollout(const l2a_mlp_shape& md, const l2a_rollout_policy& pol, int mode, int m, int n) {
    l2a_traj_plan tp = l2a_traj_plan();
    tp.deal = {0, 99, 0};
    int kind = pol.kernel_kind;
    if (kind == L2A_KERNEL_AUTO) kind = md.mfma_ok ? L2A_KERNEL_MFMA : L2A_KERNEL_VALU;
    if (kind != L2A_KERNEL_MFMA || !md.mfma_ok || !md.micro_ok) return tp;
    if (mode == L2A_MODE_PER_BLOCK && m > md.n_sets) return tp;
    const int e_loop = (mode == L2A_MODE_MEAN) ? md.n_sets : 1;
    const int cus = pol.num_cu;
    tp.deal = l2a_deal_micro(cus, m, n, 3);
    const int smem_need = l2a_mlp_micro_smem(md.H, md.KG0, md.n_hidden, e_loop);
    const long long span = (long long)((mode == L2A_MODE_PER_BLOCK ? m : e_loop) - 1) * md.set_stride * 4 +
                           l2a_mlp_micro_floats(md.H, md.KG0, md.n_hidden) * 4;
    const long long rows = (long long)m * n;
    const bool eligible = tp.deal.hi <= 3 && smem_need <= pol.lds_per_block && span < (1LL << 31) &&
                          rows * md.obs_dim * 4 < 0x7ffffff0LL && rows * md.act_dim * 4 < 0x7ffffff0LL;
    const long long tiles16 = (long long)m * ceil_div(n, 16);
    const bool measured = e_loop == 1 || 2 * tiles16 > cus;
    const bool wanted = pol.micro_policy == 2 || (pol.micro_policy == 1 && measured);
    tp.single = eligible && wanted;
    tp.gact = (!(fast_act(md.hidden_act) && fast_act(md.output_act)) || md.n_hidden == 1) ? 1 : 0;
    tp.smem = smem_need < 84 * 1024 ? 84 * 1024 : smem_need;
    tp.m_bytes = span;
    return tp;
}

int launch_rollout(l2a_model* md, L2AKParams& p, void* stream_v) {
    l2a_ctx* ctx = md->ctx;
    l2a_device_guard guard(ctx->device);
    hipStream_t stream = reinterpret_cast<hipStream_t>(stream_v);
    const int sets_needed = (p.mode == L2A_MODE_PER_BLOCK) ? (p.m < md->n_sets ? p.m : md->n_sets) : md->n_sets;
    for (int e = 0; e < sets_needed; ++e) {
        if (!md->weights_set[e]) return fail(ctx, L2A_ESTATE, "weight set " + std::to_string(e) + " was never set");
        if (!md->norm_set[e]) return fail(ctx, L2A_ESTATE, "normalisation of set " + std::to_string(e) + " was never set");
    }
    const l2a_rollout_policy pol = rollout_policy(ctx);
    l2a_rollout_plan plan;
    std::string err;
    const int prc = plan_rollout(*md, pol, {p.mode, p.m, p.n, p.h, p.obs_per_row != 0, p.state_out != nullptr,
                                            p.returns_out || p.best_key}, &plan, &err);
    if (prc != L2A_OK) return fail(ctx, prc, err);
    p.done_total = plan.done_total;
    for (int i = 0; i < plan.n_launch; ++i) {
        const l2a_rollout_launch& d = plan.launch[i];
        if (d.split) {
            const int rc = l2a_xbuf_reserve(ctx, &md->xb, plan.xbuf_bytes, stream, &p.xtag);
            if (rc != L2A_OK) return rc;
            p.xbuf = md->xb.buf;
            p.status = ctx->status_dev;
            p.spin_limit = ctx->spin_limit;
        }
        p.c_lo = d.c_lo; p.c_hi = d.c_hi;
        p.sa_elems = d.sa_elems; p.tiles_per_env = d.tiles_per_env;
        p.cst_set = d.cst_set; p.n_cst = d.n_cst; p.lb = d.lb; p.cst_off = d.cst_off;
        p.split = d.split; p.split_from = d.split_from;
        p.pl_units = d.pl_units; p.pl_f = d.pl_f; p.pl_r = d.pl_r; p.pl_w = d.pl_w;
        p.mc_w = d.mc_w; p.mc_hi = d.mc_hi; p.mc_r = d.mc_r; p.m_bytes = d.m_bytes;
        p.dbg = (plan.n_launch == 1 || (i == 0) == pol.dbg_front) ? ctx->dbg : nullptr;
        if (d.family == L2A_FAMILY_MFMA16) {
            const bool dbl = d.geo == 2 && d.nt == 2;
            const int rc = l2a_launch_mfma(d.nt, md->TPW, md->OT, md->KG0, d.gact, d.geo, &p, d.grid, d.smem, stream);
            if (rc == -100) return fail(ctx, L2A_EINVAL, dbl ? "no whole-tile MFMA kernel instance for this (obs_dim, act_dim, hidden)"
                                                             : "no MFMA kernel instance for this (obs_dim, act_dim, hidden)");
            if (rc != 0) return fail(ctx, L2A_EHIP, std::string(dbl ? "MFMA kernel launch (double rounds): " : "MFMA kernel launch: ") +
                                                        hipGetErrorString((hipError_t)rc));
        } else if (d.family == L2A_FAMILY_MICRO) {
            const int rc = l2a_launch_mlp_micro(md->H, d.gact, &p, d.grid, d.smem, stream);
            if (rc != 0) return fail(ctx, L2A_EHIP, std::string("micro-tile MLP kernel launch: ") +
                                                        (rc > 0 ? hipGetErrorString((hipError_t)rc) : "no instance"));
        } else {
            const int rc = allow_big_lds(ctx, l2a_rollout_valu_k, d.smem);
            if (rc != L2A_OK) return rc;
// ... 38 lines not shown
    }
    if (md.mfma_ok) {
        o->pk_w0 = take(packed_floats(md.in_dim, md.H));
        o->pk_wmid_stride = packed_floats(md.H, md.H);
        o->pk_wmid = take(o->pk_wmid_stride * (md.n_hidden - 1));
        o->pk_wout = take(packed_floats(md.H, md.obs_dim));
        if (md.micro_ok) o->pk_m = take(l2a_mlp_micro_floats(md.H, md.KG0, md.n_hidden));
    }
    o->pk_bout = take(16 * md.OT);
    o->nm_off = take(32 * md.KG0 + 32 * md.OT);
    return off;
}

void fill_model_params(const l2a_model* md, L2AKParams& p) {
    std::memset(&p, 0, sizeof(p));
    p.wblk = md->wblk;
    p.set_stride = md->set_stride;
    for (int i = 0; i < L2A_MAX_LAYERS; ++i) {
        p.raw_w[i] = md->raw_w[i];
        p.raw_b[i] = md->raw_b[i];
        p.hidden[i] = md->hidden[i];
    }
    p.pk_w0 = md->pk_w0; p.pk_wmid = md->pk_wmid; p.pk_wmid_stride = md->pk_wmid_stride;
    p.pk_wout = md->pk_wout; p.pk_bout = md->pk_bout; p.nm_off = md->nm_off;
    p.pk_m = md->pk_m; p.m_o4 = md->m_o4;
    p.m_nrec = md->micro_ok ? l2a_mlp_micro_nrec(md->H, md->KG0, md->n_hidden) : 0;
    p.n_hidden = md->n_hidden;
    p.obs_dim = md->obs_dim; p.act_dim = md->act_dim; p.in_dim = md->in_dim;
    p.hidden_act = md->hidden_act; p.output_act = md->output_act;
    p.mode = md->mode; p.n_sets = md->n_sets;
    p.KG0 = md->KG0; p.OT = md->OT; p.hmax = md->hmax;
    p.hid_floor = (md->hidden_act == L2A_ACT_RELU) ? 0.0f : -INFINITY;
    p.out_floor = (md->output_act == L2A_ACT_RELU) ? 0.0f : -INFINITY;
}

}

extern "C" {

int l2a_init(int device, l2a_ctx** out) {
    if (!out) return fail(nullptr, L2A_EINVAL, "l2a_init: out is null");
    *out = nullptr;
    int count = 0;
    hipError_t e = hipGetDeviceCount(&count);
    if (e != hipSuccess || count <= 0)
        return fail(nullptr, L2A_ENODEV, std::string("no HIP device visible: ") +
                                             (e != hipSuccess ? hipGetErrorString(e) : "device count is 0"));
    if (device < 0 || device >= count)
        return fail(nullptr, L2A_EINVAL, "device index " + std::to_string(device) + " out of range");
    hipDeviceProp_t prop;
    e = hipGetDeviceProperties(&prop, device);
    if (e != hipSuccess) return fail(nullptr, L2A_EHIP, std::string("hipGetDeviceProperties: ") + hipGetErrorString(e));
    std::string arch(prop.gcnArchName);
    if (arch.rfind("gfx950", 0) != 0)
        return fail(nullptr, L2A_ENODEV, "libl2a_hip.so is built for gfx950 only; device reports " + arch);
    e = hipSetDevice(device);
    if (e != hipSuccess) return fail(nullptr, L2A_EHIP, std::string("hipSetDevice: ") + hipGetErrorString(e));
    l2a_ctx* ctx = new l2a_ctx();
    ctx->device = device;
    ctx->num_cu = prop.multiProcessorCount;
    ctx->lds_per_block = (int)prop.sharedMemPerBlock;
    if (ctx->lds_per_block < 160 * 1024) ctx->lds_per_block = 160 * 1024;
    ctx->clock_khz = prop.clockRate;
    ctx->arch = arch;
    ctx->name = prop.name;
    e = hipHostMalloc(reinterpret_cast<void**>(&ctx->status_host), sizeof(unsigned int), hipHostMallocMapped);
    if (e == hipSuccess) {
        *ctx->status_host = 0;
        e = hipHostGetDevicePointer(reinterpret_cast<void**>(&ctx->status_dev), ctx->status_host, 0);
    }
    if (e != hipSuccess) {
        std::string msg = std::string("allocating the launch status word: ") + hipGetErrorString(e);
        delete ctx;
        return fail(nullptr, L2A_EHIP, msg);
    }
    const char* sp = std::getenv("L2A_SPLIT");
    if (sp && sp[0] >= '0' && sp[0] <= '2') ctx->split_policy = sp[0] - '0';
    const char* xa = std::getenv("L2A_XCD_ALIGN");
    if (xa && (xa[0] == '0' || xa[0] == '1')) ctx->xcd_align = xa[0] - '0';
    const char* fn = std::getenv("L2A_FAN");
    if (fn && (fn[0] == '0' || fn[0] == '1')) ctx->fan_policy = fn[0] - '0';
    const char* db = std::getenv("L2A_DOUBLE");
    if (db && (db[0] == '0' || db[0] == '1')) ctx->double_policy = db[0] - '0';
    const char* bs = std::getenv("L2A_BATCH");
    if (bs && bs[0] >= '0' && bs[0] <= '4') ctx->batch_sets = bs[0] - '0';
    const char* mc = std::getenv("L2A_MICRO");
    if (mc && mc[0] >= '0' && mc[0] <= '2') ctx->micro_policy = mc[0] - '0';
    *out = ctx;
    return L2A_OK;
}

void l2a_destroy(l2a_ctx* ctx) {
    if (!ctx) return;
    (void)l2a_comm_destroy(ctx);
    if (ctx->status_host) (void)hipHostFree(ctx->status_host);
    if (ctx->mail_host) (void)hipHostFree(ctx->mail_host);
    if (ctx->done_ctr) (void)hipFree(ctx->done_ctr);
    if (ctx->key_ring) (void)hipFree(ctx->key_ring);
    delete ctx;
}

int l2a_plan_geometry(int obs_dim, int act_dim, int n_hidden, const int* hidden, int n_sets, int mode, int m, int n, int h,
                      const int* policy, int* out) {
    if (!hidden || !out || obs_dim < 1 || act_dim < 1 || n_hidden < 1 || n_hidden > L2A_MAX_LAYERS - 1 || n_sets < 1 || m < 1 || n < 1 || h < 1)
        return L2A_EINVAL;
    l2a_ctx ctx;
    ctx.num_cu = 256;
    ctx.lds_per_block = 160 * 1024;
    if (policy) {
        if (policy[0] >= 0) ctx.split_policy = policy[0];
        if (policy[1] >= 0) ctx.fan_policy = policy[1];
        if (policy[2] >= 0) ctx.micro_policy = policy[2];
        if (policy[3] > 0) ctx.num_cu = policy[3];
        if (policy[4] >= 0) ctx.double_policy = policy[4];
    }
    l2a_mlp_shape md;
    model_shape(&md, obs_dim, act_dim, n_hidden, hidden, L2A_ACT_RELU, L2A_ACT_IDENTITY, n_sets, mode);
    l2a_rollout_plan plan;
    std::string err;
    const int rc = plan_rollout(md, rollout_policy(&ctx), {mode, m, n, h, false, false, true}, &plan, &err);
    if (rc != L2A_OK) return rc;
    const l2a_rollout_launch& d = plan.launch[plan.n_launch - 1];
    const bool mfma16 = d.family == L2A_FAMILY_MFMA16;
    const int g[12] = {d.family, d.nt, d.split, mfma16 ? d.split_from : -1, d.geo == 1, (int)d.grid, d.smem, mfma16 ? d.lb : 1,
                       d.mc_hi, d.pl_units, plan.n_launch == 2 ? (int)plan.launch[0].grid : 0, d.geo == 2};
    std::memcpy(out, g, sizeof(g));
    return L2A_OK;
}

int l2a_mlp_traj_geometry(int obs_dim, int act_dim, int n_hidden, int hidden, int mode, int n_sets, int m, int n, int h,
                          int micro_policy, int num_cu, int* out) {
    if (!out || obs_dim < 1 || act_dim < 1 || n_hidden < 1 || n_hidden > L2A_MAX_LAYERS - 1 || hidden < 1 || n_sets < 1 ||
        m < 1 || n < 1 || h < 1 || micro_policy < 0 || micro_policy > 2)
        return L2A_EINVAL;
    if (mode != L2A_MODE_SINGLE && mode != L2A_MODE_PER_BLOCK && mode != L2A_MODE_MEAN) return L2A_EINVAL;
    if ((long long)m * n > 0x3fffffffLL || (mode == L2A_MODE_PER_BLOCK && m > n_sets)) return L2A_EINVAL;
    l2a_ctx ctx;
    ctx.num_cu = num_cu > 0 ? num_cu : 256;
    ctx.lds_per_block = 160 * 1024;
    ctx.micro_policy = micro_policy;
    int widths[L2A_MAX_LAYERS];
    for (int i = 0; i < L2A_MAX_LAYERS; ++i) widths[i] = hidden;
    l2a_mlp_shape md;
    model_shape(&md, obs_dim, act_dim, n_hidden, widths, L2A_ACT_RELU, L2A_ACT_IDENTITY, n_sets, mode);
    md.set_stride = layout_weight_set(md, nullptr);
    const l2a_traj_plan tp = plan_traj_rollout(md, rollout_policy(&ctx), mode, m, n);
    for (int i = 0; i < 8; ++i) out[i] = 0;
    out[0] = tp.single ? 1 : 0;
    out[1] = tp.single ? 1 : h;
    out[2] = tp.single ? m * tp.deal.W : m * ceil_div(n, 16);
    out[3] = tp.single ? tp.deal.W : 0;
    out[4] = tp.deal.hi;
    out[5] = tp.single ? tp.deal.mc_r : 0;
    return L2A_OK;
}

int l2a_set_split(l2a_ctx* ctx, int policy) {
    if (!ctx) return L2A_EINVAL;
    if (policy < 0 || policy > 2) return fail(ctx, L2A_EINVAL, "split policy must be 0, 1 or 2");
    ctx->split_policy = policy;
    return L2A_OK;
}

int l2a_set_fan(l2a_ctx* ctx, int on) {
    if (!ctx) return L2A_EINVAL;
    if (on != 0 && on != 1) return fail(ctx, L2A_EINVAL, "member fan must be 0 or 1");
    ctx->fan_policy = on;
    return L2A_OK;
}

int l2a_set_double_rounds(l2a_ctx* ctx, int on) {
    if (!ctx) return L2A_EINVAL;
    if (on != 0 && on != 1) return fail(ctx, L2A_EINVAL, "double rounds must be 0 or 1");
    ctx->double_policy = on;
    return L2A_OK;
}

int l2a_set_batch(l2a_ctx* ctx, int sets) {
    if (!ctx) return L2A_EINVAL;
    if (sets < 0 || sets > 4) return fail(ctx, L2A_EINVAL, "sets per batch must be 0 (automatic) .. 4");
    ctx->batch_sets = sets;
    return L2A_OK;
}

int l2a_set_micro(l2a_ctx* ctx, int policy) {
    if (!ctx) return L2A_EINVAL;
    if (policy < 0 || policy > 2) return fail(ctx, L2A_EINVAL, "micro-tile policy must be 0, 1 or 2");
    ctx->micro_policy = policy;
    return L2A_OK;
}

int l2a_set_xcd_align(l2a_ctx* ctx, int on) {
    if (!ctx) return L2A_EINVAL;
    if (on != 0 && on != 1) return fail(ctx, L2A_EINVAL, "xcd alignment must be 0 or 1");
    ctx->xcd_align = on;
    return L2A_OK;
}

int l2a_inject_status(l2a_ctx* ctx, int bits) {
    if (!ctx) return L2A_EINVAL;
    *ctx->status_host |= (unsigned int)bits;
    return L2A_OK;
}

int l2a_set_spin_limit(l2a_ctx* ctx, unsigned int polls) {
    if (!ctx) return L2A_EINVAL;
    ctx->spin_limit = polls ? polls : (1u << 18);
    return L2A_OK;
}

int l2a_set_debug_buffer(l2a_ctx* ctx, void* device_ptr) {
    if (!ctx) return L2A_EINVAL;
    ctx->dbg = static_cast<unsigned long long*>(device_ptr);
    return L2A_OK;
}

int l2a_launch_status(l2a_ctx* ctx, int* status_out) {
    if (!ctx || !status_out) return L2A_EINVAL;
    *status_out = (int)(*ctx->status_host);
    *ctx->status_host = 0;
    return L2A_OK;
}

const char* l2a_last_error(const l2a_ctx* ctx) { return ctx ? ctx->err.c_str() : g_init_error.c_str(); }

int l2a_device_info(const l2a_ctx* ctx, char* buf, int cap) {
    if (!ctx || !buf || cap <= 0) return L2A_EINVAL;
    std::snprintf(buf, (size_t)cap,
                  "{\"device\": %d, \"name\": \"%s\", \"arch\": \"%s\", \"compute_units\": %d, "
                  "\"clock_khz\": %d, \"lds_per_block\": %d}",
                  ctx->device, ctx->name.c_str(), ctx->arch.c_str(), ctx->num_cu, ctx->clock_khz,
                  ctx->lds_per_block);
    return L2A_OK;
}

int l2a_set_kernel(l2a_ctx* ctx, int kind) {
    if (!ctx) return L2A_EINVAL;
    if (kind != L2A_KERNEL_AUTO && kind != L2A_KERNEL_MFMA && kind != L2A_KERNEL_VALU)
        return fail(ctx, L2A_EINVAL, "unknown kernel kind");
    ctx->kernel_kind = kind;
    return L2A_OK;
}

int l2a_mfma_eligible(int obs_dim, int act_dim, int n_hidden, const int* hidden) {
    return (hidden && mfma_eligible(obs_dim, act_dim, n_hidden, hidden)) ? 1 : 0;
}

long long l2a_packed_layer_floats(int k_in, int n_out) { return packed_floats(k_in, n_out); }

int l2a_pack_layer_host(const float* w, int k_in, int n_out, float* out) {
// ... 1275 lines not shown
```

learning_to_adapt_amd/csrc/l2a_host.h:

```cpp
#pragma once

#include <hip/hip_runtime.h>

#include <cstdlib>
#include <ctime>
#include <string>

#include "../../include/l2a.h"

#define L2A_MAIL_KEYS 64
#define L2A_MAIL_OBS 4096
struct l2a_mail {
    unsigned long long seq;
    unsigned long long keys[L2A_MAIL_KEYS];
    float obs[2][L2A_MAIL_OBS];
};

struct l2a_ctx {
    int device = 0;
    int kernel_kind = L2A_KERNEL_AUTO;
    int split_policy = 1;
    int xcd_align = 1;
    int fan_policy = 1;
    int double_policy = 1;
    int batch_sets = 0;
    int micro_policy = 1;
    unsigned int* status_host = nullptr;
    unsigned int* status_dev = nullptr;
    unsigned long long* dbg = nullptr;
    unsigned int spin_limit = 1u << 18;
    struct l2a_mail* mail_host = nullptr;
    struct l2a_mail* mail_dev = nullptr;
    unsigned int* done_ctr = nullptr;
    unsigned long long* key_ring = nullptr;
    int ring_dirty[2] = {L2A_MAIL_KEYS, L2A_MAIL_KEYS};
    unsigned long long mail_seq = 0;
    double sync_ema_us = 0.0;
    double stamps_us[6] = {0, 0, 0, 0, 0, 0};
    unsigned long long sync_shape = 0;
    void* comm = nullptr;
    int comm_rank = 0, comm_world = 0;
    int num_cu = 0;
    int cem_steps_in_flight = 0, rs_steps_in_flight = 0;
    int lds_per_block = 0;
    int clock_khz = 0;
    std::string arch;
    std::string name;
    mutable std::string err;
};

int l2a_fail(const l2a_ctx* ctx, int code, const std::string& msg);

#define L2A_HIP(ctx, call)                                                                        \
    do {                                                                                          \
        hipError_t e_ = (call);                                                                   \
        if (e_ != hipSuccess)                                                                     \
            return l2a_fail((ctx), L2A_EHIP, std::string(#call) + ": " + hipGetErrorString(e_));  \
    } while (0)

inline int l2a_ceil_div(int a, int b) { return (a + b - 1) / b; }

inline hipError_t l2a_xbuf_alloc(void** ptr, size_t bytes) {
    static int mode = -1;
    if (mode < 0) {
        const char* e = std::getenv("L2A_XBUF_MODE");
        mode = (e && (e[0] == '1' || e[0] == '3')) ? e[0] - '0' : 0;
    }
    if (mode == 0) return hipMalloc(ptr, bytes);
    return hipExtMallocWithFlags(ptr, bytes, mode == 1 ? hipDeviceMallocFinegrained : hipDeviceMallocUncached);
}

struct l2a_xbuf {
    unsigned long long* buf = nullptr;
    long long bytes = 0;
    unsigned int nonce = 0;
};
inline int l2a_xbuf_reserve(const l2a_ctx* ctx, l2a_xbuf* x, long long need, hipStream_t stream, unsigned int* xtag) {
    if (need > x->bytes) {
        if (x->buf) { L2A_HIP(ctx, hipStreamSynchronize(stream)); L2A_HIP(ctx, hipFree(x->buf)); x->buf = nullptr; }
        L2A_HIP(ctx, l2a_xbuf_alloc(reinterpret_cast<void**>(&x->buf), (size_t)need));
        L2A_HIP(ctx, hipMemsetAsync(x->buf, 0, (size_t)need, stream));
        x->bytes = need;
        x->nonce = 0;
    }
    x->nonce += 1;
    if (x->nonce >= (1u << 20)) {
        L2A_HIP(ctx, hipMemsetAsync(x->buf, 0, (size_t)x->bytes, stream));
        x->nonce = 1;
    }
    *xtag = x->nonce << 12;
    return L2A_OK;
}

struct l2a_micro_deal { int W, hi, mc_r; };
inline l2a_micro_deal l2a_deal_micro(int cus, int m, int n, int max_hi, bool rounds = false) {
    const int quads = l2a_ceil_div(n, 4);
    int W = cus / m;
    if (W > quads) W = quads;
    int hi = W > 0 ? l2a_ceil_div(quads, W) : 99;
    if (hi > max_hi && rounds) hi = max_hi;
    if (hi <= max_hi) {
        W = l2a_ceil_div(quads, hi);
        hi = l2a_ceil_div(quads, W);
    }
    return {W, hi, quads - W * (hi - 1)};
}

// ... 67 lines not shown
```

learning_to_adapt_amd/csrc/l2a_mfma.h:

```cpp
#pragma once

#include <type_traits>

#include "l2a_kernels.h"

#ifndef L2A_XEARLY
#define L2A_XEARLY 1
#endif

#ifndef L2A_NW
#define L2A_NW 4
#endif

typedef unsigned int u32x4 __attribute__((ext_vector_type(4)));
__device__ __forceinline__ __amdgpu_buffer_rsrc_t l2a_rsrc(const void* base, long long bytes) {
    return __builtin_amdgcn_make_buffer_rsrc(const_cast<void*>(base), 0, (int)bytes, 0x00020000);
}
__device__ __forceinline__ f32x4 l2a_ldw(__amdgpu_buffer_rsrc_t rs, int voff, int soff) {
    return __builtin_bit_cast(f32x4, __builtin_amdgcn_raw_buffer_load_b128(rs, voff, soff, 0));
}

template <bool GACT>
__device__ __forceinline__ f32x4 l2a_actv(f32x4 v, int kind, float floor) {
    if (GACT) return l2a_act4(v, kind);
// ... 54 lines not shown
    }
#define L2A_STAGE_S(CA, CB, FA, FB, SOFF, IMM, GF)                                         \
    {                                                                                      \
        int so_ = sb + (SOFF);                                                             \
        L2A_OPAQUE_S(so_);                                                                 \
        _Pragma("unroll") for (int tt = 0; tt < TW; ++tt)                                  \
            FA[tt] = l2a_ldw(rs, lane16 + (IMM), so_ + tt * (HT * 1024));                  \
        L2A_STAGE_REST(CA, CB, FB, GF, TW)                                                 \
    }
#define L2A_PFT_MAX 6
#define L2A_PFT(TW_, OT_) ((OT_) <= 2 ? ((TW_) < L2A_PFT_MAX ? (TW_) : L2A_PFT_MAX) : ((TW_) < 2 ? (TW_) : 2))

template <int NT, int TW, int TPW, int OT, bool LAST>
__device__ __forceinline__ void l2a_hidden_gemm(__amdgpu_buffer_rsrc_t rs, __amdgpu_buffer_rsrc_t rsn,
                                                int sb, int sbn, int twn,
                                                int tile0, const f32x4* hin,
                                                f32x4 (&aA)[TPW], f32x4 (&aB)[TPW],
                                                f32x4 (&pfO)[TPW][OT], f32x4 (&acc)[NT][TPW], int lane, int lane16,
                                                const float* bias_lds, f32x4 (&bias)[TPW], const int (&olane)[OT]) {
    constexpr int HT = L2A_NW * TPW;
    static_assert(HT % 4 == 0, "the k-group pipeline is unrolled by 4");
    f32x4 aC[TW], aD[TW], bA[NT], bB[NT], bC[NT], bD[NT];
#pragma unroll
    for (int nt = 0; nt < NT; ++nt) {
        bA[nt] = hin[(nt * HT + 0) * 64 + lane];
        bB[nt] = hin[(nt * HT + 1) * 64 + lane];
#pragma unroll
        for (int tt = 0; tt < TW; ++tt) acc[nt][tt] = (f32x4){0.f, 0.f, 0.f, 0.f};
    }
#pragma unroll
    for (int nt = 0; nt < NT; ++nt) { L2A_OPAQUE(bA[nt]); L2A_OPAQUE(bB[nt]); }
    __builtin_amdgcn_sched_barrier(0);

#pragma unroll 1
    for (int g = 0; g < HT - 4; g += 4) {
        const int soff = (g + 2) * 1024;
        L2A_STAGE_S(aA, bA, aC, bC, soff, 0, g + 2)
        L2A_STAGE_S(aB, bB, aD, bD, soff, 1024, g + 3)
        L2A_STAGE_S(aC, bC, aA, bA, soff, 2048, g + 4)
        L2A_STAGE_S(aD, bD, aB, bB, soff, 3072, g + 5)
    }
    L2A_STAGE_S(aA, bA, aC, bC, (HT - 2) * 1024, 0, HT - 2)
    L2A_STAGE_S(aB, bB, aD, bD, (HT - 2) * 1024, 1024, HT - 1)
    {
        int so_ = LAST ? tile0 * 1024 : sbn;
        L2A_OPAQUE_S(so_);
        if (LAST) {
#pragma unroll
            for (int tt = 0; tt < L2A_PFT(TW, OT); ++tt)
#pragma unroll
                for (int c = 0; c < OT; ++c)
                    if (((tt * OT + c) & 1) == 0)
                        pfO[tt][c] = l2a_ldw(rsn, olane[c], so_ + (tt + c * HT) * 1024);
        } else {
#pragma unroll
            for (int tt = 0; tt < TPW; ++tt)
                if (tt < twn) aA[tt] = l2a_ldw(rsn, lane16, so_ + tt * (HT * 1024));
        }
        L2A_STAGE_MFMA(aC, bC)
        __builtin_amdgcn_sched_barrier(0);
    }
    {
#pragma unroll
        for (int tt = 0; tt < TW; ++tt) bias[tt] = *reinterpret_cast<const f32x4*>(bias_lds + 16 * tt);
        int so_ = LAST ? tile0 * 1024 : sbn;
        L2A_OPAQUE_S(so_);
        if (LAST) {
#pragma unroll
            for (int tt = 0; tt < L2A_PFT(TW, OT); ++tt)
#pragma unroll
                for (int c = 0; c < OT; ++c)
                    if (((tt * OT + c) & 1) == 1)
                        pfO[tt][c] = l2a_ldw(rsn, olane[c], so_ + (tt + c * HT) * 1024);
        } else {
#pragma unroll
            for (int tt = 0; tt < TPW; ++tt)
                if (tt < twn) aB[tt] = l2a_ldw(rsn, lane16 + 1024, so_ + tt * (HT * 1024));
        }
        L2A_STAGE_MFMA(aD, bD)
        __builtin_amdgcn_sched_barrier(0);
    }
}

template <int NT, int TW, int TPW, int OT, int NPF, bool O4, class PF>
__device__ __forceinline__ void l2a_out_phase(const f32x4 (&hreg)[NT][TPW], f32x4 (&pfO)[TPW][OT],
                                              __amdgpu_buffer_rsrc_t rs_out, int tile0, PF prefetch,
                                              f32x4* pbuf, int chunk0, int lane, const int (&olane)[OT]) {
    constexpr int HT = L2A_NW * TPW;
    constexpr int CS = TPW / 2;
    constexpr int NCH = TW / CS;
    f32x4 a[TW][OT];
    int so_ = tile0 * 1024;
    L2A_OPAQUE_S(so_);
#pragma unroll
    for (int tt = 0; tt < TW; ++tt)
#pragma unroll
        for (int c = 0; c < OT; ++c)
            a[tt][c] = (tt < L2A_PFT(TW, OT)) ? pfO[tt][c]
                                              : l2a_ldw(rs_out, olane[c], so_ + (tt + c * HT) * 1024);
    prefetch();
    f32x4 acc[NCH][NT][OT];
#pragma unroll
    for (int ch = 0; ch < NCH; ++ch)
#pragma unroll
        for (int nt = 0; nt < NT; ++nt)
#pragma unroll
            for (int c = 0; c < OT; ++c) acc[ch][nt][c] = (f32x4){0.f, 0.f, 0.f, 0.f};
#pragma unroll
    for (int t2 = 0; t2 < CS; ++t2)
#pragma unroll
        for (int ii = 0; ii < 4; ++ii)
#pragma unroll
            for (int ch = 0; ch < NCH; ++ch)
#pragma unroll
                for (int nt = 0; nt < NT; ++nt)
#pragma unroll
                    for (int c = 0; c < OT; ++c)
                        acc[ch][nt][c] = (O4 && c == OT - 1)
                            ? L2A_MFMA4(a[ch * CS + t2][c][ii], hreg[nt][ch * CS + t2][ii], acc[ch][nt][c])
                            : L2A_MFMA(a[ch * CS + t2][c][ii], hreg[nt][ch * CS + t2][ii], acc[ch][nt][c]);
    {
        constexpr int NLATE = (TW - L2A_PFT(TW, OT)) * OT;
        constexpr int NMFMA = TW * 4 * NT * OT;
#pragma unroll
        for (int i = 0; i < NLATE; ++i) {
            __builtin_amdgcn_sched_group_barrier(0x020, 1, 0);
            __builtin_amdgcn_sched_group_barrier(0x008, 2, 0);
        }
        constexpr int PER = (NMFMA - 2 * NLATE) / NPF > 0 ? (NMFMA - 2 * NLATE) / NPF : 1;
#pragma unroll
        for (int i = 0; i < NPF; ++i) {
            __builtin_amdgcn_sched_group_barrier(0x008, PER, 0);
            __builtin_amdgcn_sched_group_barrier(0x020, 1, 0);
        }
    }
#pragma unroll
    for (int nt = 0; nt < NT; ++nt)
#pragma unroll
        for (int c = 0; c < OT; ++c)
            pbuf[((chunk0 * NT + nt) * OT + c) * 64 + lane] = (NCH == 2) ? acc[0][nt][c] + acc[NCH - 1][nt][c] : acc[0][nt][c];
}

template <int NT, int TPW, int OT, int KG0, bool GACT, int K0L = 4, bool N1 = false, bool O4 = false, bool FAN = false, bool WHOLE = false>
__global__ void __launch_bounds__(64 * L2A_NW) l2a_rollout_mfma_k(const L2AKParams p) {
    static_assert(!(FAN && WHOLE), "an instance is general, member fan or whole-tiles-only");
    constexpr bool NOHALF = FAN || WHOLE;
    constexpr int HT = L2A_NW * TPW;
    constexpr int TH = TPW / 2;
    static_assert(TPW % 2 == 0, "half members split a wave's tiles in two");
    constexpr int CST_BOUT = 32 * KG0 + 32 * OT;
    constexpr int CST_BHID = CST_BOUT + 16 * OT;
    constexpr int PS = L2A_NW * NT * OT * 64;
    const int NRM_SET = p.cst_set;
    const int LB = p.lb;
    extern __shared__ __attribute__((aligned(16))) char l2a_smem[];
    f32x4* buf0 = reinterpret_cast<f32x4*>(l2a_smem);
    f32x4* buf1 = buf0 + p.sa_elems;
    f32x4* pbase = buf0 + (LB > 1 ? LB : 2) * p.sa_elems;
    float* nrm = reinterpret_cast<float*>(buf0 + p.cst_off);

    const int tid = threadIdx.x;
    const int lane = tid & 63;
    const int wave = __builtin_amdgcn_readfirstlane(tid >> 6);
    const int jc = lane & 15;
    const int qq = lane >> 4;
    const int c0 = wave * TPW;
    int olane[OT];
#pragma unroll
    for (int c = 0; c < OT; ++c) olane[c] = ((O4 && c == OT - 1) ? ((lane & 48) | (lane & 3)) : lane) * 16;

    const int tail = p.split_from >= 0;
    const int in_tail = tail && (int)blockIdx.x >= p.split_from;
    const int split = FAN ? 3 : WHOLE ? 0 : (tail ? (in_tail ? p.split : 0) : p.split);
    const int n_tiles = p.m * p.tiles_per_env;
    const int n_pairs = tail ? n_tiles - p.split_from : n_tiles;
    int bid, grp, lpair, pairid;
    if (!tail && p.pl_units > 0) {
        const int hx = (int)blockIdx.x & 7, idx = (int)blockIdx.x >> 3;
        const int xcd = hx;
        const int f = p.pl_f, wide = p.pl_r * (f + 1);
        int u, k, xu;
        if (xcd < wide) { u = xcd / (f + 1); k = xcd - u * (f + 1); xu = f + 1; }
        else { const int y = xcd - wide; u = y / f; k = y - u * f; u += p.pl_r; xu = f; }
        const int su = (p.pl_w + xu - 1) / xu;
        const int j = k * su + idx;
        if (idx >= su || j >= p.pl_w) return;
        if (p.mode == L2A_MODE_PER_BLOCK) {
            grp = split ? j / p.tiles_per_env : 0;
            lpair = u * p.tiles_per_env + (j - grp * p.tiles_per_env);
        } else {
            grp = u;
            lpair = j;
        }
        bid = grp * n_pairs + lpair;
        pairid = lpair;
    } else if (!tail) {
        bid = l2a_logical_wg(blockIdx.x, gridDim.x);
        grp = split ? (bid / n_pairs) : 0;
        lpair = bid - grp * n_pairs;
        pairid = lpair;
    } else if (!in_tail) {
        bid = l2a_logical_wg(blockIdx.x, p.split_from);
        grp = 0; lpair = 0; pairid = bid;
    } else {
        bid = (int)blockIdx.x - p.split_from;
        grp = bid & 1; lpair = bid >> 1;
        pairid = p.split_from + lpair;
    }
#if defined(L2A_TIMELINE) || defined(L2A_WGREC)
    unsigned long long wg_t0_, wg_r0_;
    asm volatile("s_memtime %0\n\ts_memrealtime %1\n\ts_waitcnt lgkmcnt(0)" : "=s"(wg_t0_), "=s"(wg_r0_) : : "memory");
#endif
    const int env = pairid / p.tiles_per_env;
    const int tb = pairid - env * p.tiles_per_env;
    const int R = p.m * p.n;
    const int obs_dim = p.obs_dim, act_dim = p.act_dim;
    const int n_hidden = N1 ? 1 : p.n_hidden;

    int cand[NT], row[NT];
    bool valid[NT];
#pragma unroll
    for (int nt = 0; nt < NT; ++nt) {
        cand[nt] = p.c_lo + tb * (16 * NT) + nt * 16 + jc;
        valid[nt] = cand[nt] < p.c_hi;
        row[nt] = env * p.n + (valid[nt] ? cand[nt] : p.c_hi - 1);
    }

    const bool per_block = (p.mode == L2A_MODE_PER_BLOCK);
    const int e_loop = (p.mode == L2A_MODE_MEAN) ? p.n_sets : 1;
    const int e_half = (e_loop + 1) >> 1;
    const int e_shared = (!NOHALF && split == 2) ? e_half - 1 : -1;
    const int n_full = FAN ? 1 : (!split ? e_loop : (grp == 0 ? e_half - (split == 2 ? 1 : 0) : e_loop - e_half));
    const int n_seq = FAN ? 1 : n_full + (split == 2 ? 1 : 0);
    const int full0 = FAN ? grp : ((split && grp == 1) ? e_half : 0);
    auto seq = [&](int i) { return (i < n_full) ? full0 + i : e_shared; };
    auto set_base = [&](int e) { return p.wblk + (long long)(per_block ? env : e) * p.set_stride; };

    f32x4* xlds = reinterpret_cast<f32x4*>(nrm + p.n_cst * NRM_SET);
    for (int i = tid; i < n_seq * NRM_SET; i += 64 * L2A_NW) {
        const int s = i / NRM_SET;
        const int o = i - s * NRM_SET;
        const float* src = set_base(seq(s));
        float v;
        if (o < CST_BOUT) v = src[p.nm_off + o];
        else if (o < CST_BHID) v = src[p.pk_bout + (o - CST_BOUT)];
        else {
            const int l = (o - CST_BHID) / (16 * HT);
            v = src[p.raw_b[l] + (o - CST_BHID - l * 16 * HT)];
        }
        nrm[i] = v;
    }

    f32x4 st[NT][OT];
#pragma unroll
    for (int nt = 0; nt < NT; ++nt) {
        const float* orow = p.obs0 + (p.obs_per_row ? (long long)row[nt] : (long long)env) * obs_dim;
#pragma unroll
        for (int c = 0; c < OT; ++c)
#pragma unroll
            for (int ii = 0; ii < 4; ++ii) {
                const int dim = 16 * c + 4 * qq + ii;
                const float v = orow[dim < obs_dim ? dim : obs_dim - 1];
                st[nt][c][ii] = (dim < obs_dim) ? v : 0.0f;
            }
    }
    __syncthreads();

    const int ga0 = obs_dim >> 4;
    f32x4 av_next[NT][2];
    int aoff[NT][2][4];
#pragma unroll
    for (int nt = 0; nt < NT; ++nt)
#pragma unroll
        for (int s = 0; s < 2; ++s)
#pragma unroll
            for (int ii = 0; ii < 4; ++ii) {
                const int ka = 16 * (ga0 + s) + 4 * qq + ii - obs_dim;
                const bool in = (ka >= 0) && (ka < act_dim);
                aoff[nt][s][ii] = in ? (row[nt] * act_dim + ka) * 4 : 0x7ffffff0;
            }
    const long long a_step = (long long)R * act_dim;
    auto load_actions = [&](int t, f32x4 (&dst)[NT][2]) {
        const __amdgpu_buffer_rsrc_t ars = l2a_rsrc(p.actions + (long long)t * a_step, a_step * 4);
#pragma unroll
        for (int nt = 0; nt < NT; ++nt)
#pragma unroll
            for (int s = 0; s < 2; ++s)
#pragma unroll
                for (int ii = 0; ii < 4; ++ii)
                    dst[nt][s][ii] = __builtin_bit_cast(float, __builtin_amdgcn_raw_buffer_load_b32(ars, aoff[nt][s][ii], 0, 0));
    };
    f32x4 av[NT][2];
    float asq[NT];
    auto take_actions = [&](int t_fetch) {
#pragma unroll
        for (int nt = 0; nt < NT; ++nt) {
            av[nt][0] = av_next[nt][0];
            av[nt][1] = av_next[nt][1];
            float s = 0.0f;
#pragma unroll
            for (int ii = 0; ii < 4; ++ii) {
                s = fmaf(av[nt][0][ii], av[nt][0][ii], s);
                s = fmaf(av[nt][1][ii], av[nt][1][ii], s);
            }
            asq[nt] = s;
        }
        load_actions((t_fetch < p.h) ? t_fetch : p.h - 1, av_next);
    };
    load_actions(0, av_next);
    take_actions(1);

    float ret[NT];
#pragma unroll
    for (int nt = 0; nt < NT; ++nt) ret[nt] = p.ret_in ? p.ret_in[(long long)env * p.n + (valid[nt] ? cand[nt] : p.c_hi - 1)] : 0.0f;

    f32x4* hcur = buf0;
// ... 184 lines not shown
                    for (int g = 0; g < KG0; ++g) {
                        mu[g] = *reinterpret_cast<const f32x4*>(nr + 16 * g + 4 * qq);
                        iv[g] = *reinterpret_cast<const f32x4*>(nr + 16 * KG0 + 16 * g + 4 * qq);
                    }
                    __builtin_amdgcn_sched_barrier(0);
#pragma unroll
                    for (int g = 0; g < KG0; ++g) norm_in(g, mu[g], iv[g], xin[XPRE ? g : 0]);
                }
                f32x4 bias0[TPW];
#pragma unroll
                for (int tt = 0; tt < TPW; ++tt)
                    bias0[tt] = *reinterpret_cast<const f32x4*>(nr + CST_BHID + 16 * (c0 + tt) + 4 * qq);
                f32x4 acc[NT][TPW];
                auto l0_mfma = [&](auto npf_tag) {
                    constexpr int NPF = decltype(npf_tag)::value;
#pragma unroll
                    for (int nt = 0; nt < NT; ++nt)
#pragma unroll
                        for (int tt = 0; tt < TPW; ++tt) acc[nt][tt] = (f32x4){0.f, 0.f, 0.f, 0.f};
#pragma unroll
                    for (int g = 0; g < KG0; ++g) {
                        f32x4 xg[NT];
                        if (XPRE) {
#pragma unroll
                            for (int nt = 0; nt < NT; ++nt) xg[nt] = xin[XPRE ? g : 0][nt];
                        } else {
                            const f32x4 mu = *reinterpret_cast<const f32x4*>(nr + 16 * g + 4 * qq);
                            const f32x4 iv = *reinterpret_cast<const f32x4*>(nr + 16 * KG0 + 16 * g + 4 * qq);
                            norm_in(g, mu, iv, xg);
                        }
#pragma unroll
                        for (int ii = 0; ii < 4; ++ii) {
                            if (g == KG0 - 1 && ii >= K0L) continue;
#pragma unroll
                            for (int nt = 0; nt < NT; ++nt)
#pragma unroll
                                for (int tt = 0; tt < TPW; ++tt)
                                    acc[nt][tt] = L2A_MFMA(a[g][tt][ii], xg[nt][ii], acc[nt][tt]);
                        }
                    }
                    if constexpr (NPF < 0) {
                        __builtin_amdgcn_sched_group_barrier(0x008, (KG0 > 1 ? 4 : K0L) * NT * TPW, 0);
#pragma unroll
                        for (int k = 0; k < (KG0 - 2) * TPW; ++k) {
                            __builtin_amdgcn_sched_group_barrier(0x020, 1, 0);
                            __builtin_amdgcn_sched_group_barrier(0x008, 4 * NT, 0);
                        }
#pragma unroll
                        for (int k = 0; k < (KG0 > 1 ? TPW : 0); ++k) {
                            __builtin_amdgcn_sched_group_barrier(0x020, 1, 0);
                            __builtin_amdgcn_sched_group_barrier(0x008, K0L * NT, 0);
                        }
                        __builtin_amdgcn_sched_group_barrier(0x020, TPW, 0);
                        return;
                    }
                    constexpr int NM = ((KG0 - 1) * 4 + K0L) * NT * TPW;
                    constexpr int PER = NM / (NPF > 0 ? NPF : 1) > 0 ? NM / (NPF > 0 ? NPF : 1) : 1;
                    __builtin_amdgcn_sched_group_barrier(0x020, (KG0 - KG0P) * TPW, 0);
#pragma unroll
                    for (int k = 0; k < NPF; ++k) {
                        __builtin_amdgcn_sched_group_barrier(0x008, PER, 0);
                        __builtin_amdgcn_sched_group_barrier(0x020, 1, 0);
                    }
                };
                if (N1) {
                    const int so = sbase(c0 * 1024);
#pragma unroll
                    for (int tt = 0; tt < L2A_PFT(TPW, OT); ++tt)
#pragma unroll
                        for (int c = 0; c < OT; ++c)
                            pfO[tt][c] = l2a_ldw(rs_out, olane[c], so + (tt + c * HT) * 1024);
                    l0_mfma(std::integral_constant<int, L2A_PFT(TPW, OT) * OT>{});
                } else if (!last_l0) {
                    const __amdgpu_buffer_rsrc_t r0n = l2a_rsrc(set_base(seq(i + 1)) + p.pk_w0, w0_bytes);
                    if (L0RF) l0_mfma(std::integral_constant<int, -1>{});
#pragma unroll
                    for (int g = 0; g < KG0P; ++g)
#pragma unroll
                        for (int tt = 0; tt < TPW; ++tt) pfL0[g][tt] = l2a_ldw(r0n, lane16, s0 + (tt * KG0 + g) * 1024);
                    if (!L0RF) l0_mfma(std::integral_constant<int, KG0P * TPW>{});
                } else {
                    const int e0 = seq(b0);
                    const __amdgpu_buffer_rsrc_t rs1 = l2a_rsrc(set_base(e0) + p.pk_wmid, wm_bytes);
                    const bool next_half = !NOHALF && (e0 == e_shared) && n_hidden == 2;
                    const int s1 = sbase(next_half ? sbh : sbf);
                    if (next_half) {
#pragma unroll
                        for (int tt = 0; tt < TH; ++tt) {
                            pfA[tt] = l2a_ldw(rs1, lane16, s1 + tt * (HT * 1024));
                            pfB[tt] = l2a_ldw(rs1, lane16 + 1024, s1 + tt * (HT * 1024));
                        }
                        l0_mfma(std::integral_constant<int, 2 * TH>{});
                    } else {
#pragma unroll
                        for (int tt = 0; tt < TPW; ++tt) {
                            pfA[tt] = l2a_ldw(rs1, lane16, s1 + tt * (HT * 1024));
                            pfB[tt] = l2a_ldw(rs1, lane16 + 1024, s1 + tt * (HT * 1024));
                        }
                        l0_mfma(std::integral_constant<int, 2 * TPW>{});
                    }
                }
                L2A_TS(9)
#pragma unroll
                for (int tt = 0; tt < TPW; ++tt) {
#pragma unroll
                    for (int nt = 0; nt < NT; ++nt)
                        hreg[nt][tt] = l2a_actv<GACT>(acc[nt][tt] + bias0[tt], p.hidden_act, p.hid_floor);
                }
                L2A_TS(10)
                if (!N1) {
                    f32x4* hdst = (LB > 1) ? buf0 + j * p.sa_elems : hcur;
#pragma unroll
                    for (int tt = 0; tt < TPW; ++tt)
#pragma unroll
                        for (int nt = 0; nt < NT; ++nt) hdst[(nt * HT + c0 + tt) * 64 + lane] = hreg[nt][tt];
                }
                L2A_TS(1)
            };

            auto member = [&](int j, auto last_tag) {
                constexpr bool last_set = decltype(last_tag)::value;
                const int i = b0 + j;
                const int e = seq(i);
                const bool is_half = !NOHALF && last_set && (e == e_shared);
                const float* wb = set_base(e);
                const float* nr = nrm + i * NRM_SET;
                const __amdgpu_buffer_rsrc_t rs_out = l2a_rsrc(wb + p.pk_wout, wo_bytes);
                f32x4* pb = (LB > 1) ? pbase + j * PS : hoth;
                L2A_TS(2)
                if (!N1) {
                    f32x4 acc[NT][TPW], bias[TPW];
                    for (int l = 1; last_set && l < n_hidden - 1; ++l) {
                        const float* wl = wb + p.pk_wmid + (long long)(l - 1) * p.pk_wmid_stride;
                        const bool next_half = is_half && (l == n_hidden - 2);
                        l2a_hidden_gemm<NT, TPW, TPW, OT, false>(l2a_rsrc(wl, wm_bytes), l2a_rsrc(wl + p.pk_wmid_stride, wm_bytes),
                                                                 sbf, next_half ? sbh : sbf, next_half ? TH : TPW, 0,
                                                                 hcur, pfA, pfB, pfO, acc, lane, lane16,
                                                                 nr + CST_BHID + l * (16 * HT) + 16 * c0 + 4 * qq, bias, olane);
#pragma unroll
                        for (int tt = 0; tt < TPW; ++tt) {
#pragma unroll
                            for (int nt = 0; nt < NT; ++nt)
                                hoth[(nt * HT + c0 + tt) * 64 + lane] = l2a_actv<GACT>(acc[nt][tt] + bias[tt], p.hidden_act, p.hid_floor);
                        }
                        __syncthreads();
                        f32x4* tmp = hcur; hcur = hoth; hoth = tmp;
                    }
                    if (LB == 1) pb = hoth;
                    L2A_TS(15)
                    const f32x4* hin = (LB > 1) ? buf0 + j * p.sa_elems : hcur;
                    const __amdgpu_buffer_rsrc_t rs_last =
                        l2a_rsrc(wb + p.pk_wmid + (long long)(n_hidden - 2) * p.pk_wmid_stride, wm_bytes);
                    const float* bl = nr + CST_BHID + (n_hidden - 1) * (16 * HT);
                    if (!is_half) {
                        l2a_hidden_gemm<NT, TPW, TPW, OT, true>(rs_last, rs_out, sbf, sbf, TPW, c0, hin, pfA, pfB, pfO,
                                                                acc, lane, lane16, bl + 16 * c0 + 4 * qq, bias, olane);
#pragma unroll
                        for (int tt = 0; tt < TPW; ++tt) {
#pragma unroll
                            for (int nt = 0; nt < NT; ++nt)
                                hreg[nt][tt] = l2a_actv<GACT>(acc[nt][tt] + bias[tt], p.hidden_act, p.hid_floor);
                        }
                    } else {
                        l2a_hidden_gemm<NT, TH, TPW, OT, true>(rs_last, rs_out, sbh, sbh, TH, tile0h, hin, pfA, pfB,
                                                               pfO, acc, lane, lane16, bl + 16 * tile0h + 4 * qq, bias, olane);
#pragma unroll
                        for (int tt = 0; tt < TH; ++tt) {
#pragma unroll
                            for (int nt = 0; nt < NT; ++nt)
                                hreg[nt][tt] = l2a_actv<GACT>(acc[nt][tt] + bias[tt], p.hidden_act, p.hid_floor);
                        }
                    }
                }
                L2A_TS(3)
                if (last_set) {
                    const __amdgpu_buffer_rsrc_t r0n = l2a_rsrc(set_base(seq((i + 1 < n_seq) ? i + 1 : 0)) + p.pk_w0, w0_bytes);
                    auto pf_l0 = [&]() {
                        const int s0 = sbase(sb0);
#pragma unroll
                        for (int g = 0; g < KG0P; ++g)
#pragma unroll
                            for (int tt = 0; tt < TPW; ++tt) pfL0[g][tt] = l2a_ldw(r0n, lane16, s0 + (tt * KG0 + g) * 1024);
                    };
                    if (is_half) l2a_out_phase<NT, TH, TPW, OT, KG0P * TPW, O4>(hreg, pfO, rs_out, tile0h, pf_l0, pb, wave, lane, olane);
                    else l2a_out_phase<NT, TPW, TPW, OT, KG0P * TPW, O4>(hreg, pfO, rs_out, c0, pf_l0, pb, wave, lane, olane);
                } else {
                    const int en = seq(i + 1);
                    const __amdgpu_buffer_rsrc_t rsn = l2a_rsrc(set_base(en) + p.pk_wmid, wm_bytes);
                    if (!NOHALF && en == e_shared) {
                        l2a_out_phase<NT, TPW, TPW, OT, 2 * TH, O4>(hreg, pfO, rs_out, c0, [&]() {
                            const int s1 = sbase(sbh);
#pragma unroll
                            for (int tt = 0; tt < TH; ++tt) {
                                pfA[tt] = l2a_ldw(rsn, lane16, s1 + tt * (HT * 1024));
                                pfB[tt] = l2a_ldw(rsn, lane16 + 1024, s1 + tt * (HT * 1024));
                            }
                        }, pb, wave, lane, olane);
                    } else {
                        l2a_out_phase<NT, TPW, TPW, OT, 2 * TPW, O4>(hreg, pfO, rs_out, c0, [&]() {
                            const int s1 = sbase(sbf);
#pragma unroll
                            for (int tt = 0; tt < TPW; ++tt) {
                                pfA[tt] = l2a_ldw(rsn, lane16, s1 + tt * (HT * 1024));
                                pfB[tt] = l2a_ldw(rsn, lane16 + 1024, s1 + tt * (HT * 1024));
                            }
                        }, pb, wave, lane, olane);
                    }
                }
                L2A_TS(4)
            };
            for (int j = 0; j + 1 < nb; ++j) layer0(j, std::false_type{});
            layer0(nb - 1, std::true_type{});
            if (!N1) __syncthreads();
            for (int j = 0; j + 1 < nb; ++j) member(j, std::false_type{});
            member(nb - 1, std::true_type{});

            __syncthreads();
            if (b0 + nb >= n_seq) break;
            phase_c(std::false_type{});
            if (N1) { f32x4* tmp = hcur; hcur = hoth; hoth = tmp; }
        }
        const bool xearly = phase_c(std::true_type{});
        if (N1) { f32x4* tmp = hcur; hcur = hoth; hoth = tmp; }

        { const int e = 7; L2A_TS(9) }
        float asq_t[NT];
#pragma unroll
        for (int nt = 0; nt < NT; ++nt) asq_t[nt] = asq[nt];
        if (FAN) {
            constexpr int XREGF = NT * OT * 2 * 64 * 16;
            auto fbase = [&](int g) { return ((lpair * e_loop + g) * 2 + (t & 1)) * XREGF + lane * 16; };
            if (wave == 0) {
#pragma unroll
                for (int nt = 0; nt < NT; ++nt)
#pragma unroll
                    for (int c = 0; c < OT; ++c) {
#pragma unroll
                        for (int hh = 0; hh < 2; ++hh) {
                            u32x4 g;
                            g.x = xtag; g.y = __float_as_uint(dgrp[nt][c][2 * hh]);
                            g.z = xtag; g.w = __float_as_uint(dgrp[nt][c][2 * hh + 1]);
                            __builtin_amdgcn_raw_buffer_store_b128(g, xrs, fbase(grp) + ((nt * OT + c) * 2 + hh) * 1024, 0, L2A_SC1);
                        }
                        xlds[((grp * NT + nt) * OT + c) * 64 + lane] = dgrp[nt][c];
                    }
            }
            { const int e = 7; L2A_TS(11) }
            take_actions(t + 2);
            for (int k = wave; k < e_loop - 1; k += L2A_NW) {
                int g2 = grp + 1 + k;
                if (g2 >= e_loop) g2 -= e_loop;
                f32x4 oth[NT][OT];
                while (true) {
                    bool ok = true;
#pragma unroll
                    for (int nt = 0; nt < NT; ++nt)
#pragma unroll
                        for (int c = 0; c < OT; ++c)
#pragma unroll
                            for (int hh = 0; hh < 2; ++hh) {
                                const u32x4 g = __builtin_amdgcn_raw_buffer_load_b128(
                                    xrs, fbase(g2) + ((nt * OT + c) * 2 + hh) * 1024, 0, L2A_SC1);
                                oth[nt][c][2 * hh] = __uint_as_float(g.y);
                                oth[nt][c][2 * hh + 1] = __uint_as_float(g.w);
                                ok = ok && (g.x == xtag) && (g.z == xtag);
                            }
                    if (__all(ok)) break;
                    if (spin_left == 0) {
                        if (lane == 0) __hip_atomic_fetch_or(p.status, 1u, __ATOMIC_RELAXED, __HIP_MEMORY_SCOPE_SYSTEM);
                        break;
                    }
                    --spin_left;
                    __builtin_amdgcn_s_sleep(4);
                }
#pragma unroll
                for (int nt = 0; nt < NT; ++nt)
#pragma unroll
                    for (int c = 0; c < OT; ++c) xlds[((g2 * NT + nt) * OT + c) * 64 + lane] = oth[nt][c];
            }
            { const int e = 7; L2A_TS(12) }
            __syncthreads();
            { const int e = 7; L2A_TS(13) }
#pragma unroll
            for (int nt = 0; nt < NT; ++nt)
#pragma unroll
                for (int c = 0; c < OT; ++c) {
                    dsum[nt][c] = (f32x4){0.f, 0.f, 0.f, 0.f};
                    dgrp[nt][c] = (f32x4){0.f, 0.f, 0.f, 0.f};
                }
            {
                constexpr int EMAX = 8;
                f32x4 v[EMAX][NT][OT];
#pragma unroll
                for (int e = 0; e < EMAX; ++e) {
                    const int es = e < e_loop ? e : e_loop - 1;
#pragma unroll
                    for (int nt = 0; nt < NT; ++nt)
#pragma unroll
                        for (int c = 0; c < OT; ++c) v[e][nt][c] = xlds[((es * NT + nt) * OT + c) * 64 + lane];
                }
                __builtin_amdgcn_sched_barrier(0);
#pragma unroll
                for (int e = 0; e < EMAX; ++e)
#pragma unroll
                    for (int nt = 0; nt < NT; ++nt)
// ... 229 lines not shown
```

learning_to_adapt_amd/csrc/l2a_mfma_inst.hip:

```cpp
#include "l2a_mfma.h"

#ifndef L2A_INST_FAN
#define L2A_INST_FAN 0
#endif

#if !defined(L2A_INST_NT) || !defined(L2A_INST_TPW)
#error "compile with -DL2A_INST_NT=<1|2> -DL2A_INST_TPW=<2|4|8>"
#endif

namespace {

template <int OT, int KG0, bool GACT, int K0L = 4, bool N1 = false, bool O4 = false>
int launch_one(const L2AKParams* p, unsigned grid, int smem, hipStream_t stream) {
    if (!N1 && p->n_hidden == 1) return launch_one<OT, KG0, true, 4, true>(p, grid, smem, stream);
    auto kernel = l2a_rollout_mfma_k<L2A_INST_NT, L2A_INST_TPW, OT, KG0, GACT, K0L, N1, O4, L2A_INST_FAN == 1, L2A_INST_FAN == 2>;
    static int smem_set[16] = {0};
    int dev = 0;
    (void)hipGetDevice(&dev);
    if (dev < 0 || dev >= 16 || smem > smem_set[dev]) {
        hipError_t e = hipFuncSetAttribute(reinterpret_cast<const void*>(kernel),
                                           hipFuncAttributeMaxDynamicSharedMemorySize, smem);
        if (e != hipSuccess) return (int)e;
        if (dev >= 0 && dev < 16) smem_set[dev] = smem;
    }
    hipLaunchKernelGGL(kernel, dim3(grid), dim3(64 * L2A_NW), smem, stream, *p);
    return 0;
}

template <bool GACT>
int launch_shape(int ot, int kg0, const L2AKParams* p, unsigned grid, int smem, hipStream_t stream) {
    switch (ot * 8 + kg0) {
        case 1 * 8 + 1: return launch_one<1, 1, GACT>(p, grid, smem, stream);
        case 1 * 8 + 2: return launch_one<1, 2, GACT>(p, grid, smem, stream);
        case 2 * 8 + 2:
            if (p->n_hidden > 1 && p->obs_dim - 16 >= 1 && p->obs_dim - 16 <= 4)
                return launch_one<2, 2, GACT, 4, false, true>(p, grid, smem, stream);
            return launch_one<2, 2, GACT>(p, grid, smem, stream);
        case 2 * 8 + 3: return launch_one<2, 3, GACT>(p, grid, smem, stream);
        case 3 * 8 + 3: return launch_one<3, 3, GACT>(p, grid, smem, stream);
        case 3 * 8 + 4:
            if constexpr (!GACT) {
                if (p->in_dim == 49) return launch_one<3, 4, GACT, 1>(p, grid, smem, stream);
            }
            return launch_one<3, 4, GACT>(p, grid, smem, stream);
#if L2A_INST_NT == 1 && L2A_INST_FAN != 2
        case 4 * 8 + 4: return launch_one<4, 4, GACT>(p, grid, smem, stream);
        case 4 * 8 + 5: return launch_one<4, 5, GACT>(p, grid, smem, stream);
#endif
        default: return -100;
    }
}

}

#define L2A_CAT3(a, b, c) a##b##_##c
#if L2A_INST_FAN == 2
#define L2A_NAME(nt, tpw) L2A_CAT3(l2a_launch_mfma_whole_, nt, tpw)
#elif L2A_INST_FAN
#define L2A_NAME(nt, tpw) L2A_CAT3(l2a_launch_mfma_fan_, nt, tpw)
#else
#define L2A_NAME(nt, tpw) L2A_CAT3(l2a_launch_mfma_, nt, tpw)
#endif

int L2A_NAME(L2A_INST_NT, L2A_INST_TPW)(int ot, int kg0, int gact, const L2AKParams* p, unsigned grid, int smem,
                                         hipStream_t stream) {
    return gact ? launch_shape<true>(ot, kg0, p, grid, smem, stream)
                : launch_shape<false>(ot, kg0, p, grid, smem, stream);
}
```

learning_to_adapt_amd/csrc/l2a_mfma_launch.h:

```cpp
#pragma once

#include <hip/hip_runtime.h>

struct L2AKParams;

#ifndef L2A_NW
#define L2A_NW 4
#endif

#define L2A_DECL_LAUNCH(NT_, TPW_)                                                               \
    int l2a_launch_mfma_##NT_##_##TPW_(int ot, int kg0, int gact, const L2AKParams* p, unsigned grid, \
                                       int smem, hipStream_t stream);
L2A_DECL_LAUNCH(1, 2) L2A_DECL_LAUNCH(1, 4) L2A_DECL_LAUNCH(1, 8)
L2A_DECL_LAUNCH(2, 2) L2A_DECL_LAUNCH(2, 4)
L2A_DECL_LAUNCH(fan_1, 2) L2A_DECL_LAUNCH(fan_1, 4) L2A_DECL_LAUNCH(fan_1, 8) L2A_DECL_LAUNCH(fan_2, 8)
L2A_DECL_LAUNCH(whole_2, 8) L2A_DECL_LAUNCH(whole_1, 8)
#undef L2A_DECL_LAUNCH

inline int l2a_launch_mfma(int nt, int tpw, int ot, int kg0, int gact, int geo, const L2AKParams* p, unsigned grid,
                           int smem, hipStream_t stream) {
    static_assert(L2A_NW == 4, "instances are generated for 4-wave workgroups (TPW = H / 64)");
    if (geo == 2) {
        if (nt == 2 && tpw == 8) return l2a_launch_mfma_whole_2_8(ot, kg0, gact, p, grid, smem, stream);
        if (nt == 1 && tpw == 8) return l2a_launch_mfma_whole_1_8(ot, kg0, gact, p, grid, smem, stream);
        return -100;
    }
    if (geo == 1) {
        if (nt == 1 && tpw == 2) return l2a_launch_mfma_fan_1_2(ot, kg0, gact, p, grid, smem, stream);
        if (nt == 1 && tpw == 4) return l2a_launch_mfma_fan_1_4(ot, kg0, gact, p, grid, smem, stream);
        if (nt == 1 && tpw == 8) return l2a_launch_mfma_fan_1_8(ot, kg0, gact, p, grid, smem, stream);
        if (nt == 2 && tpw == 8) return l2a_launch_mfma_fan_2_8(ot, kg0, gact, p, grid, smem, stream);
        return -100;
    }
    if (nt == 1 && tpw == 2) return l2a_launch_mfma_1_2(ot, kg0, gact, p, grid, smem, stream);
    if (nt == 1 && tpw == 4) return l2a_launch_mfma_1_4(ot, kg0, gact, p, grid, smem, stream);
    if (nt == 1 && tpw == 8) return l2a_launch_mfma_1_8(ot, kg0, gact, p, grid, smem, stream);
    if (nt == 2 && tpw == 2) return l2a_launch_mfma_2_2(ot, kg0, gact, p, grid, smem, stream);
    if (nt == 2 && tpw == 4) return l2a_launch_mfma_2_4(ot, kg0, gact, p, grid, smem, stream);
    return -100;
}
```

Baseline: 712.6.

## Add static three-set MFMA rollout instance for ensemble-of-five mean mode

Adds a new kernel specialization (seq3) for NT=1, TPW=8, two hidden layers, mean mode with five ensemble members split three-per-workgroup. The layer and member loops are fully unrolled for exactly three sets, and the final cross-set reduction (phase_c) is replaced by an inline version that loads all partials and norm constants up front and overlaps the exchange puts and loads. A new half-GEMM ring routine with a peeled last iteration prefetches output weights. It is enabled by default when the geometry matches, which adds a compile-time instance and more register pressure from the hoisted partial arrays.

```diff
diff --git a/include/l2a.h b/include/l2a.h
--- a/include/l2a.h
+++ b/include/l2a.h
@@ -84,6 +84,7 @@
 int l2a_set_xcd_align(l2a_ctx* ctx, int on);
 int l2a_set_fan(l2a_ctx* ctx, int on);
 int l2a_set_double_rounds(l2a_ctx* ctx, int on);
+int l2a_set_seq3(l2a_ctx* ctx, int on);
 int l2a_set_micro(l2a_ctx* ctx, int policy);
 int l2a_launch_status(l2a_ctx* ctx, int* status_out);
 int l2a_set_spin_limit(l2a_ctx* ctx, unsigned int polls);
@@ -460,6 +461,8 @@
 
 int l2a_plan_geometry(int obs_dim, int act_dim, int n_hidden, const int* hidden, int n_sets, int mode, int m, int n, int h,
                       const int* policy, int* out);
+int l2a_plan_geometry_ex(int obs_dim, int act_dim, int n_hidden, const int* hidden, int n_sets, int mode, int m, int n, int h,
+                         const int* policy, int n_policy, int* out, int n_out);
 int l2a_lstm_plan_geometry(int obs_dim, int act_dim, int n_layers, const int* units, int cell_type, int m, int n, int h, int request,
                            const int* policy, int* out);
 int l2a_mfma_eligible(int obs_dim, int act_dim, int n_hidden, const int* hidden);
diff --git a/learning_to_adapt_amd/_lib.py b/learning_to_adapt_amd/_lib.py
--- a/learning_to_adapt_amd/_lib.py
+++ b/learning_to_adapt_amd/_lib.py
@@ -22,13 +22,13 @@
 CELL_CODES = {"lstm": 0, "gru": 1, "rnn": 2}
 
 EXPORTED_SYMBOLS = (
-    "l2a_init", "l2a_destroy", "l2a_last_error", "l2a_device_info", "l2a_set_kernel", "l2a_set_split", "l2a_set_batch", "l2a_set_xcd_align", "l2a_set_fan", "l2a_set_double_rounds", "l2a_set_micro",
+    "l2a_init", "l2a_destroy", "l2a_last_error", "l2a_device_info", "l2a_set_kernel", "l2a_set_split", "l2a_set_batch", "l2a_set_xcd_align", "l2a_set_fan", "l2a_set_double_rounds", "l2a_set_seq3", "l2a_set_micro",
     "l2a_launch_status", "l2a_set_debug_buffer", "l2a_set_spin_limit", "l2a_inject_status",
     "l2a_model_create", "l2a_model_destroy", "l2a_model_set_weights", "l2a_model_set_weights_strided",
     "l2a_model_set_norm", "l2a_model_adapt_sgd", "l2a_model_adapt_sgd_host", "l2a_model_adapt_sgd_raw", "l2a_model_get_weights",
     "l2a_plan_rs", "l2a_plan_rs_sync", "l2a_plan_rs_chunk", "l2a_reward_program_check", "l2a_score_trajectory", "l2a_plan_rs_program",
     "l2a_reward_model_check", "l2a_reward_model_geometry", "l2a_reward_model_create", "l2a_reward_model_destroy", "l2a_reward_model_set_weights", "l2a_reward_model_set_norm",
-    "l2a_reward_model_predict", "l2a_score_trajectory_model", "l2a_plan_rs_reward_model", "l2a_predict", "l2a_key_encode", "l2a_key_decode", "l2a_mfma_eligible", "l2a_plan_geometry",
+    "l2a_reward_model_predict", "l2a_score_trajectory_model", "l2a_plan_rs_reward_model", "l2a_predict", "l2a_key_encode", "l2a_key_decode", "l2a_mfma_eligible", "l2a_plan_geometry", "l2a_plan_geometry_ex",
     "l2a_packed_layer_floats", "l2a_pack_layer_host", "l2a_micro_layout_floats", "l2a_micro_pack_layer_host",
     "l2a_comm_unique_id", "l2a_comm_init", "l2a_comm_destroy", "l2a_allreduce_best", "l2a_plan_payload",
     "l2a_cem_sample", "l2a_cem_refit", "l2a_cem_pick", "l2a_cem_refit_sample", "l2a_cem_refit_sample_fused",
@@ -87,18 +87,22 @@
     return dict(single=bool(v[0]), launches=v[1], workgroups=v[2], workgroups_per_env=v[3], micro_tiles=v[4], full_workgroups=v[5])
 
 
-def plan_geometry(obs_dim, act_dim, hidden, n_sets, mode, m, n, h, split=-1, fan=-1, micro=-1, cus=0, double=-1):
+def plan_geometry(obs_dim, act_dim, hidden, n_sets, mode, m, n, h, split=-1, fan=-1, micro=-1, cus=0, double=-1, batch=-1, seq3=-1):
     lib = load()
     hid = (ctypes.c_int * len(hidden))(*[int(x) for x in hidden])
-    pol = (ctypes.c_int * 5)(int(split), int(fan), int(micro), int(cus), int(double))
-    out = (ctypes.c_int * 12)()
-    rc = lib.l2a_plan_geometry(int(obs_dim), int(act_dim), len(hidden), hid, int(n_sets), MODE_CODES[mode], int(m), int(n), int(h), pol, out)
+    pol = (ctypes.c_int * 7)(int(split), int(fan), int(micro), int(cus), int(double), int(batch), int(seq3))
+    out = (ctypes.c_int * 13)()
+    if hasattr(lib, "l2a_plan_geometry_ex"):
+        rc = lib.l2a_plan_geometry_ex(int(obs_dim), int(act_dim), len(hidden), hid, int(n_sets), MODE_CODES[mode], int(m), int(n), int(h),
+                                      pol, 7, out, 13)
+    else:
+        rc = lib.l2a_plan_geometry(int(obs_dim), int(act_dim), len(hidden), hid, int(n_sets), MODE_CODES[mode], int(m), int(n), int(h), pol, out)
     if rc != L2A_OK:
         raise L2AError("l2a_plan_geometry failed (%d)" % rc)
     v = list(out)
     return dict(kernel=("valu", "mfma16", "micro")[v[0]], nt=v[1], split=v[2], split_from=v[3], fan=bool(v[4]), workgroups=v[5],
                 lds_bytes=v[6], sets_per_batch=v[7], micro_tiles=v[8], placement_units=v[9], front_workgroups=v[10],
-                whole_instance=bool(v[11]))
+                whole_instance=bool(v[11]), seq3=bool(v[12]))
 
 
 LSTM_FAMILIES = ("lstm_valu", "lstm_mfma16", "lstm_micro", "lstm_micro_traj", "generic_valu", "generic_mfma16", "generic_micro")
@@ -229,6 +233,11 @@
     else:
         lib.l2a_set_fan.argtypes = [vp, i32]
         lib.l2a_set_fan.restype = i32
+    if os.environ.get("L2A_LIB_PATH") and not hasattr(lib, "l2a_set_seq3"):
+        lib.l2a_set_seq3 = lambda handle, on: 0
+    else:
+        lib.l2a_set_seq3.argtypes = [vp, i32]
+        lib.l2a_set_seq3.restype = i32
     if os.environ.get("L2A_LIB_PATH") and not hasattr(lib, "l2a_set_double_rounds"):
         lib.l2a_set_double_rounds = lambda handle, on: 0
     else:
@@ -360,6 +369,9 @@
     lib.l2a_mfma_eligible.restype = i32
     lib.l2a_plan_geometry.argtypes = [i32, i32, i32, c.POINTER(i32), i32, i32, i32, i32, i32, c.POINTER(i32), c.POINTER(i32)]
     lib.l2a_plan_geometry.restype = i32
+    if hasattr(lib, "l2a_plan_geometry_ex") or not os.environ.get("L2A_LIB_PATH"):
+        lib.l2a_plan_geometry_ex.argtypes = [i32, i32, i32, c.POINTER(i32), i32, i32, i32, i32, i32, c.POINTER(i32), i32, c.POINTER(i32), i32]
+        lib.l2a_plan_geometry_ex.restype = i32
     lib.l2a_packed_layer_floats.argtypes = [i32, i32]
     lib.l2a_packed_layer_floats.restype = c.c_longlong
     lib.l2a_pack_layer_host.argtypes = [c.POINTER(f32), i32, i32, c.POINTER(f32)]
@@ -649,6 +661,9 @@
     def set_fan(self, on):
         self.check(self.lib.l2a_set_fan(self.handle, int(bool(on))), "l2a_set_fan")
 
+    def set_seq3(self, on):
+        self.check(self.lib.l2a_set_seq3(self.handle, int(bool(on))), "l2a_set_seq3")
+
     def set_double_rounds(self, on):
         self.check(self.lib.l2a_set_double_rounds(self.handle, int(bool(on))), "l2a_set_double_rounds")
 
diff --git a/learning_to_adapt_amd/csrc/build.py b/learning_to_adapt_amd/csrc/build.py
--- a/learning_to_adapt_amd/csrc/build.py
+++ b/learning_to_adapt_amd/csrc/build.py
@@ -16,6 +16,7 @@
 INSTANCES = [(1, 2), (1, 4), (1, 8), (2, 2), (2, 4)]
 FAN_INSTANCES = [(1, 2), (1, 4), (1, 8), (2, 8)]
 WHOLE_INSTANCES = [(2, 8), (1, 8)]
+SEQ3_INSTANCES = [(1, 8)]
 LSTM_INSTANCES = [2, 4, 8]
 FLAGS = ["--offload-arch=gfx950", "-O3", "-std=c++17", "-fPIC"]
 KERNEL_FLAGS = ["-mllvm", "--amdgpu-mfma-vgpr-form"]
@@ -102,6 +103,9 @@
     for nt, tpw in WHOLE_INSTANCES:
         t["l2a_mfma_whole_%d_%d.o" % (nt, tpw)] = ("l2a_mfma_inst.hip", ["-DL2A_INST_NT=%d" % nt, "-DL2A_INST_TPW=%d" % tpw,
                                                                           "-DL2A_INST_FAN=2"] + KERNEL_FLAGS)
+    for nt, tpw in SEQ3_INSTANCES:
+        t["l2a_mfma_seq3_%d_%d.o" % (nt, tpw)] = ("l2a_mfma_inst.hip", ["-DL2A_INST_NT=%d" % nt, "-DL2A_INST_TPW=%d" % tpw,
+                                                                         "-DL2A_INST_FAN=3"] + KERNEL_FLAGS)
     return t
 
 
@@ -149,7 +153,7 @@
     for o, (src, flags) in table.items():
         obj = os.path.join(OBJ_DIR, o)
         if only is not None and o.startswith("l2a_mfma_") and os.path.exists(obj) and \
-                tuple(int(x) for x in o[len("l2a_mfma_"):-2].replace("fan_", "").replace("whole_", "").split("_")) not in only:
+                tuple(int(x) for x in o[len("l2a_mfma_"):-2].replace("fan_", "").replace("whole_", "").replace("seq3_", "").split("_")) not in only:
             continue
         if not force and only is None and _obj_fresh(obj):
             continue
diff --git a/learning_to_adapt_amd/csrc/l2a_api.hip b/learning_to_adapt_amd/csrc/l2a_api.hip
--- a/learning_to_adapt_amd/csrc/l2a_api.hip
+++ b/learning_to_adapt_amd/csrc/l2a_api.hip
@@ -108,7 +108,7 @@
 
 
 struct l2a_rollout_policy {
-    int kernel_kind, split_policy, fan_policy, double_policy, micro_policy, batch_sets, xcd_align;
+    int kernel_kind, split_policy, fan_policy, double_policy, micro_policy, batch_sets, xcd_align, seq3_policy;
     int num_cu, lds_per_block;
     int force_nt;
     bool dbg_front;
@@ -118,7 +118,7 @@
     static const int force_nt = [] { const char* e = std::getenv("L2A_FORCE_NT"); return (e && (e[0] == '1' || e[0] == '2')) ? e[0] - '0' : 0; }();
     static const bool dbg_front = [] { const char* e = std::getenv("L2A_DBG_FRONT"); return e && e[0] == '1'; }();
     return {ctx->kernel_kind, ctx->split_policy, ctx->fan_policy, ctx->double_policy, ctx->micro_policy, ctx->batch_sets,
-            ctx->xcd_align, ctx->num_cu > 0 ? ctx->num_cu : 256, ctx->lds_per_block, force_nt, dbg_front};
+            ctx->xcd_align, ctx->seq3_policy, ctx->num_cu > 0 ? ctx->num_cu : 256, ctx->lds_per_block, force_nt, dbg_front};
 }
 
 struct l2a_rollout_request {
@@ -340,7 +340,9 @@
     d.grid = (unsigned)n_wg;
     const bool whole1 = !fan && pol.double_policy != 0 && e_loop == 1 && nt == 1 && md.TPW == 8 && md.OT <= 3 &&
                         d.split == 0 && d.split_from < 0;
-    d.geo = fan ? 1 : whole1 ? 2 : 0;
+    const bool seq3 = pol.seq3_policy != 0 && !fan && !whole1 && !gact && nt == 1 && md.TPW == 8 && md.OT <= 2 && md.KG0 <= 2 &&
+                      md.n_hidden == 2 && rq.mode == L2A_MODE_MEAN && e_loop == 5 && d.split == 2 && d.split_from < 0 && d.lb == 3;
+    d.geo = fan ? 1 : whole1 ? 2 : seq3 ? 3 : 0;
     if (front_k) plan->done_total = (int)(front.grid + pairs);
     return L2A_OK;
 }
@@ -545,6 +547,8 @@
     if (fn && (fn[0] == '0' || fn[0] == '1')) ctx->fan_policy = fn[0] - '0';
     const char* db = std::getenv("L2A_DOUBLE");
     if (db && (db[0] == '0' || db[0] == '1')) ctx->double_policy = db[0] - '0';
+    const char* s3 = std::getenv("L2A_SEQ3");
+    if (s3 && (s3[0] == '0' || s3[0] == '1')) ctx->seq3_policy = s3[0] - '0';
     const char* bs = std::getenv("L2A_BATCH");
     if (bs && bs[0] >= '0' && bs[0] <= '4') ctx->batch_sets = bs[0] - '0';
     const char* mc = std::getenv("L2A_MICRO");
@@ -565,18 +569,24 @@
 
 int l2a_plan_geometry(int obs_dim, int act_dim, int n_hidden, const int* hidden, int n_sets, int mode, int m, int n, int h,
                       const int* policy, int* out) {
+    return l2a_plan_geometry_ex(obs_dim, act_dim, n_hidden, hidden, n_sets, mode, m, n, h, policy, policy ? 5 : 0, out, 12);
+}
+
+int l2a_plan_geometry_ex(int obs_dim, int act_dim, int n_hidden, const int* hidden, int n_sets, int mode, int m, int n, int h,
+                         const int* policy, int n_policy, int* out, int n_out) {
+    if (n_policy < 0 || n_policy > 7 || n_out < 12 || n_out > 13 || (n_policy > 0 && !policy)) return L2A_EINVAL;
     if (!hidden || !out || obs_dim < 1 || act_dim < 1 || n_hidden < 1 || n_hidden > L2A_MAX_LAYERS - 1 || n_sets < 1 || m < 1 || n < 1 || h < 1)
         return L2A_EINVAL;
     l2a_ctx ctx;
     ctx.num_cu = 256;
     ctx.lds_per_block = 160 * 1024;
-    if (policy) {
-        if (policy[0] >= 0) ctx.split_policy = policy[0];
-        if (policy[1] >= 0) ctx.fan_policy = policy[1];
-        if (policy[2] >= 0) ctx.micro_policy = policy[2];
-        if (policy[3] > 0) ctx.num_cu = policy[3];
-        if (policy[4] >= 0) ctx.double_policy = policy[4];
-    }
+    if (n_policy > 0 && policy[0] >= 0) ctx.split_policy = policy[0];
+    if (n_policy > 1 && policy[1] >= 0) ctx.fan_policy = policy[1];
+    if (n_policy > 2 && policy[2] >= 0) ctx.micro_policy = policy[2];
+    if (n_policy > 3 && policy[3] > 0) ctx.num_cu = policy[3];
+    if (n_policy > 4 && policy[4] >= 0) ctx.double_policy = policy[4];
+    if (n_policy > 5 && policy[5] >= 0) ctx.batch_sets = policy[5];
+    if (n_policy > 6 && policy[6] >= 0) ctx.seq3_policy = policy[6];
     l2a_mlp_shape md;
     model_shape(&md, obs_dim, act_dim, n_hidden, hidden, L2A_ACT_RELU, L2A_ACT_IDENTITY, n_sets, mode);
     l2a_rollout_plan plan;
@@ -585,9 +595,9 @@
     if (rc != L2A_OK) return rc;
     const l2a_rollout_launch& d = plan.launch[plan.n_launch - 1];
     const bool mfma16 = d.family == L2A_FAMILY_MFMA16;
-    const int g[12] = {d.family, d.nt, d.split, mfma16 ? d.split_from : -1, d.geo == 1, (int)d.grid, d.smem, mfma16 ? d.lb : 1,
-                       d.mc_hi, d.pl_units, plan.n_launch == 2 ? (int)plan.launch[0].grid : 0, d.geo == 2};
-    std::memcpy(out, g, sizeof(g));
+    const int g[13] = {d.family, d.nt, d.split, mfma16 ? d.split_from : -1, d.geo == 1, (int)d.grid, d.smem, mfma16 ? d.lb : 1,
+                       d.mc_hi, d.pl_units, plan.n_launch == 2 ? (int)plan.launch[0].grid : 0, d.geo == 2, d.geo == 3};
+    std::memcpy(out, g, sizeof(int) * n_out);
     return L2A_OK;
 }
 
@@ -629,6 +639,13 @@
     if (!ctx) return L2A_EINVAL;
     if (on != 0 && on != 1) return fail(ctx, L2A_EINVAL, "member fan must be 0 or 1");
     ctx->fan_policy = on;
+    return L2A_OK;
+}
+
+int l2a_set_seq3(l2a_ctx* ctx, int on) {
+    if (!ctx) return L2A_EINVAL;
+    if (on != 0 && on != 1) return fail(ctx, L2A_EINVAL, "static three-set step must be 0 or 1");
+    ctx->seq3_policy = on;
     return L2A_OK;
 }
 
diff --git a/learning_to_adapt_amd/csrc/l2a_host.h b/learning_to_adapt_amd/csrc/l2a_host.h
--- a/learning_to_adapt_amd/csrc/l2a_host.h
+++ b/learning_to_adapt_amd/csrc/l2a_host.h
@@ -23,6 +23,7 @@
     int xcd_align = 1;
     int fan_policy = 1;
     int double_policy = 1;
+    int seq3_policy = 1;
     int batch_sets = 0;
     int micro_policy = 1;
     unsigned int* status_host = nullptr;
diff --git a/learning_to_adapt_amd/csrc/l2a_mfma.h b/learning_to_adapt_amd/csrc/l2a_mfma.h
--- a/learning_to_adapt_amd/csrc/l2a_mfma.h
+++ b/learning_to_adapt_amd/csrc/l2a_mfma.h
@@ -160,6 +160,75 @@
     }
 }
 
+template <int NT, int TPW, int OT>
+__device__ __forceinline__ void l2a_half_gemm_ring(__amdgpu_buffer_rsrc_t rs, __amdgpu_buffer_rsrc_t rsn, int sb, int tile0,
+                                                   const f32x4* hin, const f32x4 (&pfA)[TPW], const f32x4 (&pfB)[TPW],
+                                                   f32x4 (&pfO)[TPW][OT], f32x4 (&acc)[NT][TPW], int lane, int lane16,
+                                                   const float* bias_lds, f32x4 (&bias)[TPW], const int (&olane)[OT]) {
+    constexpr int HT = L2A_NW * TPW;
+    constexpr int TW = TPW / 2;
+    static_assert(HT % 8 == 0 && HT >= 16, "the ring is unrolled by 8 and its last iteration is peeled");
+    f32x4 a[8][TW], b[4][NT];
+#pragma unroll
+    for (int tt = 0; tt < TW; ++tt) {
+        a[0][tt] = pfA[tt]; a[1][tt] = pfB[tt];
+        a[2][tt] = pfA[TW + tt]; a[3][tt] = pfB[TW + tt];
+    }
+#pragma unroll
+    for (int nt = 0; nt < NT; ++nt) {
+        b[0][nt] = hin[(nt * HT + 0) * 64 + lane];
+        b[1][nt] = hin[(nt * HT + 1) * 64 + lane];
+#pragma unroll
+        for (int tt = 0; tt < TW; ++tt) acc[nt][tt] = (f32x4){0.f, 0.f, 0.f, 0.f};
+    }
+#pragma unroll
+    for (int nt = 0; nt < NT; ++nt) { L2A_OPAQUE(b[0][nt]); L2A_OPAQUE(b[1][nt]); }
+    __builtin_amdgcn_sched_barrier(0);
+
+#pragma unroll 1
+    for (int g = 0; g < HT - 8; g += 8) {
+        const int soff = (g + 4) * 1024;
+        L2A_STAGE_S(a[0], b[0], a[4], b[2], soff, 0, g + 2)
+        L2A_STAGE_S(a[1], b[1], a[5], b[3], soff, 1024, g + 3)
+        L2A_STAGE_S(a[2], b[2], a[6], b[0], soff, 2048, g + 4)
+        L2A_STAGE_S(a[3], b[3], a[7], b[1], soff, 3072, g + 5)
+        L2A_STAGE_S(a[4], b[0], a[0], b[2], soff + 4096, 0, g + 6)
+        L2A_STAGE_S(a[5], b[1], a[1], b[3], soff + 4096, 1024, g + 7)
+        L2A_STAGE_S(a[6], b[2], a[2], b[0], soff + 4096, 2048, g + 8)
+        L2A_STAGE_S(a[7], b[3], a[3], b[1], soff + 4096, 3072, g + 9)
+    }
+    L2A_STAGE_S(a[0], b[0], a[4], b[2], (HT - 4) * 1024, 0, HT - 6)
+    L2A_STAGE_S(a[1], b[1], a[5], b[3], (HT - 4) * 1024, 1024, HT - 5)
+    L2A_STAGE_S(a[2], b[2], a[6], b[0], (HT - 4) * 1024, 2048, HT - 4)
+    L2A_STAGE_S(a[3], b[3], a[7], b[1], (HT - 4) * 1024, 3072, HT - 3)
+    { L2A_STAGE_REST(a[4], b[0], b[2], HT - 2, 0) }
+    { L2A_STAGE_REST(a[5], b[1], b[3], HT - 1, 0) }
+    {
+        int so_ = tile0 * 1024;
+        L2A_OPAQUE_S(so_);
+#pragma unroll
+        for (int tt = 0; tt < L2A_PFT(TW, OT); ++tt)
+#pragma unroll
+            for (int c = 0; c < OT; ++c)
+                if (((tt * OT + c) & 1) == 0) pfO[tt][c] = l2a_ldw(rsn, olane[c], so_ + (tt + c * HT) * 1024);
+        L2A_STAGE_MFMA(a[6], b[2])
+        __builtin_amdgcn_sched_barrier(0);
+    }
+    {
+#pragma unroll
+        for (int tt = 0; tt < TW; ++tt) bias[tt] = *reinterpret_cast<const f32x4*>(bias_lds + 16 * tt);
+        int so_ = tile0 * 1024;
+        L2A_OPAQUE_S(so_);
+#pragma unroll
+        for (int tt = 0; tt < L2A_PFT(TW, OT); ++tt)
+#pragma unroll
+            for (int c = 0; c < OT; ++c)
+                if (((tt * OT + c) & 1) == 1) pfO[tt][c] = l2a_ldw(rsn, olane[c], so_ + (tt + c * HT) * 1024);
+        L2A_STAGE_MFMA(a[7], b[3])
+        __builtin_amdgcn_sched_barrier(0);
+    }
+}
+
 template <int NT, int TW, int TPW, int OT, int NPF, bool O4, class PF>
 __device__ __forceinline__ void l2a_out_phase(const f32x4 (&hreg)[NT][TPW], f32x4 (&pfO)[TPW][OT],
                                               __amdgpu_buffer_rsrc_t rs_out, int tile0, PF prefetch,
@@ -219,9 +288,12 @@
             pbuf[((chunk0 * NT + nt) * OT + c) * 64 + lane] = (NCH == 2) ? acc[0][nt][c] + acc[NCH - 1][nt][c] : acc[0][nt][c];
 }
 
-template <int NT, int TPW, int OT, int KG0, bool GACT, int K0L = 4, bool N1 = false, bool O4 = false, bool FAN = false, bool WHOLE = false>
+template <int NT, int TPW, int OT, int KG0, bool GACT, int K0L = 4, bool N1 = false, bool O4 = false, bool FAN = false, bool WHOLE = false,
+          bool SEQ3 = false>
 __global__ void __launch_bounds__(64 * L2A_NW) l2a_rollout_mfma_k(const L2AKParams p) {
     static_assert(!(FAN && WHOLE), "an instance is general, member fan or whole-tiles-only");
+    static_assert(!SEQ3 || (L2A_XEARLY && !FAN && !WHOLE && !N1 && NT == 1 && TPW == 8 && OT <= 2 && KG0 <= 2),
+                  "the static three-set step exists for the (1, 8) tile-split shapes of the early exchange");
     constexpr bool NOHALF = FAN || WHOLE;
     constexpr int HT = L2A_NW * TPW;
     constexpr int TH = TPW / 2;
@@ -230,7 +302,7 @@
     constexpr int CST_BHID = CST_BOUT + 16 * OT;
     constexpr int PS = L2A_NW * NT * OT * 64;
     const int NRM_SET = p.cst_set;
-    const int LB = p.lb;
+    const int LB = SEQ3 ? 3 : p.lb;
     extern __shared__ __attribute__((aligned(16))) char l2a_smem[];
     f32x4* buf0 = reinterpret_cast<f32x4*>(l2a_smem);
     f32x4* buf1 = buf0 + p.sa_elems;
@@ -247,9 +319,9 @@
 #pragma unroll
     for (int c = 0; c < OT; ++c) olane[c] = ((O4 && c == OT - 1) ? ((lane & 48) | (lane & 3)) : lane) * 16;
 
-    const int tail = p.split_from >= 0;
+    const int tail = SEQ3 ? 0 : p.split_from >= 0;
     const int in_tail = tail && (int)blockIdx.x >= p.split_from;
-    const int split = FAN ? 3 : WHOLE ? 0 : (tail ? (in_tail ? p.split : 0) : p.split);
+    const int split = SEQ3 ? 2 : FAN ? 3 : WHOLE ? 0 : (tail ? (in_tail ? p.split : 0) : p.split);
     const int n_tiles = p.m * p.tiles_per_env;
     const int n_pairs = tail ? n_tiles - p.split_from : n_tiles;
     int bid, grp, lpair, pairid;
@@ -293,7 +365,7 @@
     const int tb = pairid - env * p.tiles_per_env;
     const int R = p.m * p.n;
     const int obs_dim = p.obs_dim, act_dim = p.act_dim;
-    const int n_hidden = N1 ? 1 : p.n_hidden;
+    const int n_hidden = N1 ? 1 : SEQ3 ? 2 : p.n_hidden;
 
     int cand[NT], row[NT];
     bool valid[NT];
@@ -304,12 +376,12 @@
         row[nt] = env * p.n + (valid[nt] ? cand[nt] : p.c_hi - 1);
     }
 
-    const bool per_block = (p.mode == L2A_MODE_PER_BLOCK);
-    const int e_loop = (p.mode == L2A_MODE_MEAN) ? p.n_sets : 1;
+    const bool per_block = !SEQ3 && (p.mode == L2A_MODE_PER_BLOCK);
+    const int e_loop = SEQ3 ? 5 : (p.mode == L2A_MODE_MEAN) ? p.n_sets : 1;
     const int e_half = (e_loop + 1) >> 1;
     const int e_shared = (!NOHALF && split == 2) ? e_half - 1 : -1;
-    const int n_full = FAN ? 1 : (!split ? e_loop : (grp == 0 ? e_half - (split == 2 ? 1 : 0) : e_loop - e_half));
-    const int n_seq = FAN ? 1 : n_full + (split == 2 ? 1 : 0);
+    const int n_full = SEQ3 ? 2 : FAN ? 1 : (!split ? e_loop : (grp == 0 ? e_half - (split == 2 ? 1 : 0) : e_loop - e_half));
+    const int n_seq = SEQ3 ? 3 : FAN ? 1 : n_full + (split == 2 ? 1 : 0);
     const int full0 = FAN ? grp : ((split && grp == 1) ? e_half : 0);
     auto seq = [&](int i) { return (i < n_full) ? full0 + i : e_shared; };
     auto set_base = [&](int e) { return p.wblk + (long long)(per_block ? env : e) * p.set_stride; };
@@ -660,7 +732,7 @@
                 } else {
                     const int e0 = seq(b0);
                     const __amdgpu_buffer_rsrc_t rs1 = l2a_rsrc(set_base(e0) + p.pk_wmid, wm_bytes);
-                    const bool next_half = !NOHALF && (e0 == e_shared) && n_hidden == 2;
+                    const bool next_half = !SEQ3 && !NOHALF && (e0 == e_shared) && n_hidden == 2;
                     const int s1 = sbase(next_half ? sbh : sbf);
                     if (next_half) {
 #pragma unroll
@@ -700,7 +772,7 @@
                 constexpr bool last_set = decltype(last_tag)::value;
                 const int i = b0 + j;
                 const int e = seq(i);
-                const bool is_half = !NOHALF && last_set && (e == e_shared);
+                const bool is_half = SEQ3 ? last_set : (!NOHALF && last_set && (e == e_shared));
                 const float* wb = set_base(e);
                 const float* nr = nrm + i * NRM_SET;
                 const __amdgpu_buffer_rsrc_t rs_out = l2a_rsrc(wb + p.pk_wout, wo_bytes);
@@ -740,6 +812,10 @@
                                 hreg[nt][tt] = l2a_actv<GACT>(acc[nt][tt] + bias[tt], p.hidden_act, p.hid_floor);
                         }
                     } else {
+                        if constexpr (SEQ3)
+                            l2a_half_gemm_ring<NT, TPW, OT>(rs_last, rs_out, sbh, tile0h, hin, pfA, pfB,
+                                                            pfO, acc, lane, lane16, bl + 16 * tile0h + 4 * qq, bias, olane);
+                        else
                         l2a_hidden_gemm<NT, TH, TPW, OT, true>(rs_last, rs_out, sbh, sbh, TH, tile0h, hin, pfA, pfB,
                                                                pfO, acc, lane, lane16, bl + 16 * tile0h + 4 * qq, bias, olane);
 #pragma unroll
@@ -765,7 +841,26 @@
                 } else {
                     const int en = seq(i + 1);
                     const __amdgpu_buffer_rsrc_t rsn = l2a_rsrc(set_base(en) + p.pk_wmid, wm_bytes);
-                    if (!NOHALF && en == e_shared) {
+                    if constexpr (SEQ3) {
+                        if (j == 1) {
+                            l2a_out_phase<NT, TPW, TPW, OT, 4 * TH, O4>(hreg, pfO, rs_out, c0, [&]() {
+                                const int s1 = sbase(sbh);
+#pragma unroll
+                                for (int tt = 0; tt < TH; ++tt) {
+                                    pfA[tt] = l2a_ldw(rsn, lane16, s1 + tt * (HT * 1024));
+                                    pfB[tt] = l2a_ldw(rsn, lane16 + 1024, s1 + tt * (HT * 1024));
+                                }
+#pragma unroll
+                                for (int tt = 0; tt < TH; ++tt) {
+                                    pfA[TH + tt] = l2a_ldw(rsn, lane16 + 2048, s1 + tt * (HT * 1024));
+                                    pfB[TH + tt] = l2a_ldw(rsn, lane16 + 3072, s1 + tt * (HT * 1024));
+                                }
+                            }, pb, wave, lane, olane);
+                            L2A_TS(4)
+                            return;
+                        }
+                    }
+                    if (!SEQ3 && !NOHALF && en == e_shared) {
                         l2a_out_phase<NT, TPW, TPW, OT, 2 * TH, O4>(hreg, pfO, rs_out, c0, [&]() {
                             const int s1 = sbase(sbh);
 #pragma unroll
@@ -787,18 +882,91 @@
                 }
                 L2A_TS(4)
             };
+            if constexpr (SEQ3) {
+                layer0(0, std::false_type{});
+                layer0(1, std::false_type{});
+                layer0(2, std::true_type{});
+                __syncthreads();
+                member(0, std::false_type{});
+                member(1, std::false_type{});
+                member(2, std::true_type{});
+            } else {
             for (int j = 0; j + 1 < nb; ++j) layer0(j, std::false_type{});
             layer0(nb - 1, std::true_type{});
             if (!N1) __syncthreads();
             for (int j = 0; j + 1 < nb; ++j) member(j, std::false_type{});
             member(nb - 1, std::true_type{});
+            }
 
             __syncthreads();
             if (b0 + nb >= n_seq) break;
             phase_c(std::false_type{});
             if (N1) { f32x4* tmp = hcur; hcur = hoth; hoth = tmp; }
         }
-        const bool xearly = phase_c(std::true_type{});
+        bool xearly;
+        if constexpr (SEQ3) {
+            f32x4 part[3][OT][L2A_NW][NT], cb[2][OT], cm[2][OT], cs[2][OT];
+            { const int e = 2; L2A_TS(5) } { const int e = seq(0); L2A_TS(5) } { const int e = seq(1); L2A_TS(5) }
+#pragma unroll
+            for (int k = 0; k < 3; ++k) {
+                const int j = (k == 0) ? 2 : k - 1;
+#pragma unroll
+                for (int c = 0; c < OT; ++c)
+#pragma unroll
+                    for (int ch = 0; ch < L2A_NW; ++ch)
+#pragma unroll
+                        for (int nt = 0; nt < NT; ++nt) part[j][c][ch][nt] = pbase[j * PS + ((ch * NT + nt) * OT + c) * 64 + lane];
+            }
+#pragma unroll
+            for (int j = 0; j < 2; ++j) {
+                const float* nr = nrm + j * NRM_SET;
+#pragma unroll
+                for (int c = 0; c < OT; ++c) {
+                    cb[j][c] = *reinterpret_cast<const f32x4*>(nr + CST_BOUT + 16 * c + 4 * qq);
+                    cm[j][c] = *reinterpret_cast<const f32x4*>(nr + 32 * KG0 + 16 * c + 4 * qq);
+                    cs[j][c] = *reinterpret_cast<const f32x4*>(nr + 32 * KG0 + 16 * OT + 16 * c + 4 * qq);
+                }
+            }
+            __builtin_amdgcn_sched_barrier(0);
+#pragma unroll
+            for (int c = 0; c < OT; ++c)
+#pragma unroll
+                for (int nt = 0; nt < NT; ++nt)
+                    qsh[nt][c] = (part[2][c][0][nt] + part[2][c][1][nt]) + (part[2][c][2][nt] + part[2][c][3][nt]);
+            if (wave == 0) xput(1, qsh);
+            { const int e = 2; L2A_TS(6) }
+#pragma unroll
+            for (int j = 0; j < 2; ++j)
+#pragma unroll
+                for (int c = 0; c < OT; ++c)
+#pragma unroll
+                    for (int nt = 0; nt < NT; ++nt) {
+                        f32x4 s = (part[j][c][0][nt] + part[j][c][1][nt]) + (part[j][c][2][nt] + part[j][c][3][nt]);
+                        if (O4 && c == OT - 1) {
+#pragma unroll
+                            for (int ii = 0; ii < 4; ++ii) s[ii] = l2a_sum_xor32(l2a_sum_xor16(s[ii]));
+                        }
+                        s = l2a_actv<GACT>(s + cb[j][c], p.output_act, p.out_floor);
+                        dgrp[nt][c] += s * cs[j][c] + cm[j][c];
+                    }
+            if (wave == 1) xput(0, dgrp);
+            if (wave == 3) {
+#pragma unroll
+                for (int r = 0; r < 2; ++r)
+#pragma unroll
+                    for (int nt = 0; nt < NT; ++nt)
+#pragma unroll
+                        for (int c = 0; c < OT; ++c)
+#pragma unroll
+                            for (int hh = 0; hh < 2; ++hh)
+                                sw[r][nt][c][hh] = __builtin_amdgcn_raw_buffer_load_b128(
+                                    xrs, xbase(grp ^ 1, r) + ((nt * OT + c) * 2 + hh) * 1024, 0, L2A_SC1);
+            }
+            { const int e = seq(0); L2A_TS(6) } { const int e = seq(1); L2A_TS(6) }
+            xearly = true;
+        } else {
+            xearly = phase_c(std::true_type{});
+        }
         if (N1) { f32x4* tmp = hcur; hcur = hoth; hoth = tmp; }
 
         { const int e = 7; L2A_TS(9) }
diff --git a/learning_to_adapt_amd/csrc/l2a_mfma_inst.hip b/learning_to_adapt_amd/csrc/l2a_mfma_inst.hip
--- a/learning_to_adapt_amd/csrc/l2a_mfma_inst.hip
+++ b/learning_to_adapt_amd/csrc/l2a_mfma_inst.hip
@@ -1,4 +1,5 @@
 #include "l2a_mfma.h"
+#include "l2a_mfma_launch.h"
 
 #ifndef L2A_INST_FAN
 #define L2A_INST_FAN 0
@@ -7,13 +8,19 @@
 #if !defined(L2A_INST_NT) || !defined(L2A_INST_TPW)
 #error "compile with -DL2A_INST_NT=<1|2> -DL2A_INST_TPW=<2|4|8>"
 #endif
+#if L2A_INST_FAN == 3 && (L2A_INST_NT != 1 || L2A_INST_TPW != 8)
+#error "the static three-set step is built for NT = 1, TPW = 8"
+#endif
 
 namespace {
 
 template <int OT, int KG0, bool GACT, int K0L = 4, bool N1 = false, bool O4 = false>
 int launch_one(const L2AKParams* p, unsigned grid, int smem, hipStream_t stream) {
-    if (!N1 && p->n_hidden == 1) return launch_one<OT, KG0, true, 4, true>(p, grid, smem, stream);
-    auto kernel = l2a_rollout_mfma_k<L2A_INST_NT, L2A_INST_TPW, OT, KG0, GACT, K0L, N1, O4, L2A_INST_FAN == 1, L2A_INST_FAN == 2>;
+    if constexpr (L2A_INST_FAN != 3) {
+        if (!N1 && p->n_hidden == 1) return launch_one<OT, KG0, true, 4, true>(p, grid, smem, stream);
+    }
+    auto kernel = l2a_rollout_mfma_k<L2A_INST_NT, L2A_INST_TPW, OT, KG0, GACT, K0L, N1, O4, L2A_INST_FAN == 1, L2A_INST_FAN == 2,
+                                     L2A_INST_FAN == 3>;
     static int smem_set[16] = {0};
     int dev = 0;
     (void)hipGetDevice(&dev);
@@ -29,6 +36,19 @@
 
 template <bool GACT>
 int launch_shape(int ot, int kg0, const L2AKParams* p, unsigned grid, int smem, hipStream_t stream) {
+#if L2A_INST_FAN == 3 && !L2A_XEARLY
+    return -100;
+#elif L2A_INST_FAN == 3
+    if constexpr (GACT) return -100;
+    else switch (ot * 8 + kg0) {
+        case 1 * 8 + 1: return launch_one<1, 1, GACT>(p, grid, smem, stream);
+        case 1 * 8 + 2: return launch_one<1, 2, GACT>(p, grid, smem, stream);
+        case 2 * 8 + 2:
+            if (p->obs_dim - 16 >= 1 && p->obs_dim - 16 <= 4) return launch_one<2, 2, GACT, 4, false, true>(p, grid, smem, stream);
+            return launch_one<2, 2, GACT>(p, grid, smem, stream);
+        default: return -100;
+    }
+#else
     switch (ot * 8 + kg0) {
         case 1 * 8 + 1: return launch_one<1, 1, GACT>(p, grid, smem, stream);
         case 1 * 8 + 2: return launch_one<1, 2, GACT>(p, grid, smem, stream);
@@ -49,12 +69,15 @@
 #endif
         default: return -100;
     }
+#endif
 }
 
 }
 
 #define L2A_CAT3(a, b, c) a##b##_##c
-#if L2A_INST_FAN == 2
+#if L2A_INST_FAN == 3
+#define L2A_NAME(nt, tpw) L2A_CAT3(l2a_launch_mfma_seq3_, nt, tpw)
+#elif L2A_INST_FAN == 2
 #define L2A_NAME(nt, tpw) L2A_CAT3(l2a_launch_mfma_whole_, nt, tpw)
 #elif L2A_INST_FAN
 #define L2A_NAME(nt, tpw) L2A_CAT3(l2a_launch_mfma_fan_, nt, tpw)
@@ -64,6 +87,9 @@
 
 int L2A_NAME(L2A_INST_NT, L2A_INST_TPW)(int ot, int kg0, int gact, const L2AKParams* p, unsigned grid, int smem,
                                          hipStream_t stream) {
+#if L2A_INST_FAN == 3 && !L2A_XEARLY
+    return l2a_launch_mfma_1_8(ot, kg0, gact, p, grid, smem, stream);
+#endif
     return gact ? launch_shape<true>(ot, kg0, p, grid, smem, stream)
                 : launch_shape<false>(ot, kg0, p, grid, smem, stream);
 }
diff --git a/learning_to_adapt_amd/csrc/l2a_mfma_launch.h b/learning_to_adapt_amd/csrc/l2a_mfma_launch.h
--- a/learning_to_adapt_amd/csrc/l2a_mfma_launch.h
+++ b/learning_to_adapt_amd/csrc/l2a_mfma_launch.h
@@ -15,11 +15,13 @@
 L2A_DECL_LAUNCH(2, 2) L2A_DECL_LAUNCH(2, 4)
 L2A_DECL_LAUNCH(fan_1, 2) L2A_DECL_LAUNCH(fan_1, 4) L2A_DECL_LAUNCH(fan_1, 8) L2A_DECL_LAUNCH(fan_2, 8)
 L2A_DECL_LAUNCH(whole_2, 8) L2A_DECL_LAUNCH(whole_1, 8)
+L2A_DECL_LAUNCH(seq3_1, 8)
 #undef L2A_DECL_LAUNCH
 
 inline int l2a_launch_mfma(int nt, int tpw, int ot, int kg0, int gact, int geo, const L2AKParams* p, unsigned grid,
                            int smem, hipStream_t stream) {
     static_assert(L2A_NW == 4, "instances are generated for 4-wave workgroups (TPW = H / 64)");
+    if (geo == 3) return (nt == 1 && tpw == 8) ? l2a_launch_mfma_seq3_1_8(ot, kg0, gact, p, grid, smem, stream) : -100;
     if (geo == 2) {
         if (nt == 2 && tpw == 8) return l2a_launch_mfma_whole_2_8(ot, kg0, gact, p, grid, smem, stream);
         if (nt == 1 && tpw == 8) return l2a_launch_mfma_whole_1_8(ot, kg0, gact, p, grid, smem, stream);
```

Measured after the change: 737.0 (median of 6 runs). +3.4%, better.
